# irwenqiang/DiFacto

Measured on AMD Instinct MI355X. Metric: train examples/sec (FM V_dim=16) at 1/8 GPU + achieved HBM GB/s, higher is better.
Workload: dtype f32; 1 GPU; C3 Criteo-shaped FM V_dim=16, 39 binary nnz/row, 2^24 keys, l1=0 V_threshold=0, fused dfx_train_step; config=c3, rows_per_gpu_step=100000, global_batch=100000, parallelism=single GPU

## Files before the change

### difacto_amd/_lib.py

```python
import ctypes
import os

import torch

LIB_PATH = os.environ.get("DFX_LIB_PATH") or os.path.join(
    os.path.dirname(os.path.abspath(__file__)), "libdifacto_amd.so")

_lib = None

c_i64 = ctypes.c_int64
c_u64 = ctypes.c_uint64
vp = ctypes.c_void_p
i64p = ctypes.POINTER(ctypes.c_int64)
f64p = ctypes.POINTER(ctypes.c_double)


class DfxError(RuntimeError):
    pass


class Batch(ctypes.Structure):
    _fields_ = [("size", c_i64), ("nnz", c_i64), ("offset", vp), ("index", vp), ("value", vp),
                ("label", vp), ("weight", vp)]


class Progress(ctypes.Structure):
    _fields_ = [("nrows", ctypes.c_double), ("loss", ctypes.c_double), ("auc", ctypes.c_double),
                ("penalty", ctypes.c_double), ("nnz_w", ctypes.c_double)]


class HostBatch(ctypes.Structure):
    _fields_ = [("offset", vp), ("index", vp), ("value", vp), ("label", vp), ("weight", vp),
                ("max_rows", c_i64), ("max_nnz", c_i64)]


_SIGS = {
    "dfx_last_error": (ctypes.c_char_p, []),
    "dfx_ctx_create": (ctypes.c_int, [ctypes.c_int, ctypes.c_char_p, ctypes.POINTER(vp)]),
    "dfx_ctx_destroy": (ctypes.c_int, [vp]),
    "dfx_ctx_set_stream": (ctypes.c_int, [vp, vp]),
    "dfx_ctx_use_own_stream": (ctypes.c_int, [vp]),
    "dfx_ctx_set_input_stream": (ctypes.c_int, [vp, vp]),
    "dfx_prof_lanes": (ctypes.c_int, [vp, f64p]),
    "dfx_prof_counts": (ctypes.c_int, [vp, f64p]),
    "dfx_prof_host": (ctypes.c_int, [vp, f64p]),
    "dfx_ctx_vdim": (ctypes.c_int, [vp]),
    "dfx_sync": (ctypes.c_int, [vp]),
    "dfx_malloc": (ctypes.c_int, [vp, ctypes.POINTER(vp), ctypes.c_size_t]),
    "dfx_free": (ctypes.c_int, [vp, vp]),
    "dfx_memcpy": (ctypes.c_int, [vp, vp, vp, ctypes.c_size_t, ctypes.c_int]),
    "dfx_reserve": (ctypes.c_int, [vp, c_i64, c_i64]),
    "dfx_localize": (ctypes.c_int, [vp, c_i64, c_i64, vp, vp, c_u64, vp, vp, vp, i64p]),
    "dfx_fm_predict": (ctypes.c_int, [vp, c_i64, c_i64, vp, vp, vp, vp, vp, vp, c_i64,
                                      ctypes.c_int, vp]),
    "dfx_fm_calcgrad": (ctypes.c_int, [vp, c_i64, c_i64, vp, vp, vp, vp, vp, vp, vp, vp, c_i64,
                                       ctypes.c_int, vp, vp]),
    "dfx_get_pos": (ctypes.c_int, [vp, c_i64, vp, vp, vp]),
    "dfx_evaluate": (ctypes.c_int, [vp, c_i64, vp, vp, f64p]),
    "dfx_auc": (ctypes.c_int, [vp, c_i64, vp, vp, f64p]),
    "dfx_store_pull": (ctypes.c_int, [vp, vp, c_i64, vp, vp, i64p]),
    "dfx_store_push": (ctypes.c_int, [vp, vp, c_i64, ctypes.c_int, vp, c_i64, vp]),
    "dfx_store_save": (ctypes.c_int, [vp, ctypes.c_char_p, ctypes.c_int]),
    "dfx_store_load": (ctypes.c_int, [vp, ctypes.c_char_p]),
    "dfx_store_load_part": (ctypes.c_int, [vp, ctypes.c_char_p, ctypes.c_int, ctypes.c_int]),
    "dfx_store_dump": (ctypes.c_int, [vp, ctypes.c_char_p, ctypes.c_int, ctypes.c_int]),
    "dfx_store_stats": (ctypes.c_int, [vp, i64p, i64p, f64p, ctypes.POINTER(ctypes.c_uint32)]),
    "dfx_store_evaluate": (ctypes.c_int, [vp, f64p, i64p]),
    "dfx_store_reserve": (ctypes.c_int, [vp, c_i64, c_i64]),
    "dfx_store_entry": (ctypes.c_int, [vp, c_u64, vp, vp, ctypes.POINTER(ctypes.c_int),
                                       ctypes.POINTER(ctypes.c_int)]),
    "dfx_train_step": (ctypes.c_int, [vp, ctypes.POINTER(Batch), ctypes.c_int, ctypes.c_int,
                                      c_u64, vp]),
    "dfx_progress_read": (ctypes.c_int, [vp, ctypes.POINTER(Progress), ctypes.c_int]),
    "dfx_prof_enable": (ctypes.c_int, [vp, ctypes.c_int]),
    "dfx_prof_enable_marks": (ctypes.c_int, [vp, ctypes.c_int, ctypes.c_uint]),
    "dfx_prof_read": (ctypes.c_int, [vp, f64p, ctypes.POINTER(ctypes.c_int), f64p]),
    "dfx_feeder_create": (ctypes.c_int, [vp, c_i64, c_i64, ctypes.POINTER(vp)]),
    "dfx_feeder_destroy": (ctypes.c_int, [vp]),
    "dfx_feeder_slot": (ctypes.c_int, [vp, ctypes.POINTER(HostBatch)]),
    "dfx_feeder_submit": (ctypes.c_int, [vp, c_i64, c_i64, ctypes.c_int, ctypes.c_int,
                                         ctypes.POINTER(Batch)]),
    "dfx_feeder_consumed": (ctypes.c_int, [vp]),
    "dfx_feeder_create_slots": (ctypes.c_int, [vp, c_i64, c_i64, ctypes.c_int,
                                               ctypes.POINTER(vp)]),
    "dfx_feeder_consumed_back": (ctypes.c_int, [vp, ctypes.c_int]),
    "dfx_dist_record_floats": (ctypes.c_int, [vp]),
    "dfx_dist_localize": (ctypes.c_int, [vp, ctypes.POINTER(Batch), c_u64, ctypes.c_int,
                                         ctypes.c_int, vp, vp]),
    "dfx_dist_localize_wait": (ctypes.c_int, [vp, ctypes.c_int, ctypes.c_int, i64p, i64p]),
    "dfx_dist_owner_begin": (ctypes.c_int, [vp, ctypes.c_int, vp, i64p, ctypes.c_int, vp]),
    "dfx_dist_owner_pull": (ctypes.c_int, [vp, ctypes.c_int, vp]),
    "dfx_dist_fwd_bwd": (ctypes.c_int, [vp, ctypes.c_int, ctypes.POINTER(Batch), vp,
                                        ctypes.c_int, vp, vp]),
    "dfx_dist_owner_push": (ctypes.c_int, [vp, ctypes.c_int, vp]),
    "dfx_dist_initv_local": (ctypes.c_int, [vp, ctypes.c_int, vp]),
    "dfx_dist_initv_draw": (ctypes.c_int, [vp, ctypes.c_int, vp, ctypes.c_int, ctypes.c_int]),
    "dfx_dist_push_agg_sum": (ctypes.c_int, [vp]),
    "dfx_store_probe_stats": (ctypes.c_int, [vp, vp, vp, vp]),
    "dfx_dist_union": (ctypes.c_int, [vp, vp, vp, ctypes.c_int, ctypes.c_int, vp, vp, vp, vp]),
    "dfx_dist_union_rows": (ctypes.c_int, [vp, vp, vp, ctypes.c_int64, vp, ctypes.c_int,
                                           ctypes.c_int64, ctypes.c_int, ctypes.c_int, vp, vp]),
    "dfx_split_part_floats": (ctypes.c_int, [vp, ctypes.c_int]),
    "dfx_split_pxv_floats": (ctypes.c_int, [vp]),
    "dfx_split_partition": (ctypes.c_int, [vp, ctypes.c_int, ctypes.POINTER(Batch), c_u64,
                                           ctypes.c_int, vp, vp, vp]),
    "dfx_split_partition_wait": (ctypes.c_int, [vp, ctypes.c_int, ctypes.c_int, i64p]),
    "dfx_split_owner_begin": (ctypes.c_int, [vp, ctypes.c_int, vp, vp, vp, i64p, i64p,
                                             ctypes.c_int, ctypes.c_int, ctypes.c_int,
                                             ctypes.c_int]),
    "dfx_ctx_lane_stream": (ctypes.c_int, [vp, ctypes.c_int, ctypes.POINTER(vp)]),
    "dfx_ctx_set_lane_stream": (ctypes.c_int, [vp, ctypes.c_int, vp]),
    "dfx_split_owner_forward": (ctypes.c_int, [vp, ctypes.c_int, vp]),
    "dfx_split_owner_forward_rows": (ctypes.c_int, [vp, ctypes.c_int, vp, ctypes.c_int, c_i64,
                                                    c_i64, c_i64]),
    "dfx_split_combine_rows": (ctypes.c_int, [vp, ctypes.c_int, ctypes.POINTER(Batch), vp, c_i64,
                                              ctypes.c_int, vp, vp, c_i64, c_i64]),
    "dfx_split_combine": (ctypes.c_int, [vp, ctypes.c_int, ctypes.POINTER(Batch), vp, c_i64,
                                         ctypes.c_int, vp, vp]),
    "dfx_split_owner_backward": (ctypes.c_int, [vp, ctypes.c_int, vp]),
    "dfx_split_owner_stats": (ctypes.c_int, [vp, ctypes.c_int, i64p, i64p, i64p]),
    "dfx_split_initv_local": (ctypes.c_int, [vp, ctypes.c_int, vp]),
    "dfx_split_initv_draw": (ctypes.c_int, [vp, ctypes.c_int, vp, ctypes.c_int, ctypes.c_int]),
}

EXPORTED = tuple(_SIGS)


def lib():
    global _lib
    if _lib is None:
        if not os.path.exists(LIB_PATH):
            raise DfxError("libdifacto_amd.so is not built (%s); run `make` at the repo root"
                           % LIB_PATH)
        L = ctypes.CDLL(LIB_PATH)
        lenient = bool(os.environ.get("DFX_LIB_PATH"))
        for name, (res, args) in _SIGS.items():
            if lenient and not hasattr(L, name):
                continue
            fn = getattr(L, name)
            fn.restype = res
            fn.argtypes = args
        _lib = L
    return _lib


def check(rc):
    if rc != 0:
        msg = lib().dfx_last_error()
        raise DfxError("libdifacto_amd: status %d: %s" % (rc, msg.decode() if msg else "?"))


DIST_PATH = os.path.join(os.path.dirname(os.path.abspath(LIB_PATH)), "libdfx_dist.so")
_dist = None
u32 = ctypes.c_uint32

_DIST_SIGS = {
    "dfx_dist_last_error": (ctypes.c_char_p, []),
    "dfx_dist_rccl_id_bytes": (ctypes.c_int, []),
    "dfx_dist_rccl_ids": (ctypes.c_int, [ctypes.c_int, vp]),
    "dfx_dist_rccl_comms": (ctypes.c_int, []),
    "dfx_split_store_set_slices": (ctypes.c_int, [vp, ctypes.c_int]),
    "dfx_split_store_allreduce_sum": (ctypes.c_int, [vp, f64p, ctypes.c_int]),
    "dfx_split_store_create_rccl": (ctypes.c_int, [vp, ctypes.c_int, ctypes.c_int, vp,
                                                   ctypes.c_int, ctypes.c_int, c_u64,
                                                   ctypes.POINTER(vp)]),
    "dfx_split_store_create_loopback": (ctypes.c_int, [ctypes.POINTER(vp), ctypes.c_int,
                                                       ctypes.c_int, c_u64, ctypes.POINTER(vp)]),
    "dfx_split_store_submit": (ctypes.c_int, [vp, ctypes.POINTER(Batch), ctypes.c_int,
                                              ctypes.c_int, ctypes.POINTER(vp)]),
    "dfx_split_store_flush": (ctypes.c_int, [vp]),
    "dfx_split_store_sync": (ctypes.c_int, [vp]),
    "dfx_split_store_throttle_seconds": (ctypes.c_int, [vp, f64p]),
    "dfx_split_store_set_marks": (ctypes.c_int, [vp, u32]),
    "dfx_split_store_take_marks": (ctypes.c_int, [vp, f64p, i64p]),
    "dfx_split_store_destroy": (ctypes.c_int, [vp]),
}

DIST_EXPORTED = tuple(_DIST_SIGS)


def dist_lib():
    global _dist
    if _dist is None:
        lib()
        if not os.path.exists(DIST_PATH):
            raise DfxError("libdfx_dist.so is not built (%s); run `make` at the repo root"
                           % DIST_PATH)
        L = ctypes.CDLL(DIST_PATH)
        for name, (res, args) in _DIST_SIGS.items():
            fn = getattr(L, name)
            fn.restype = res
            fn.argtypes = args
        _dist = L
    return _dist


def dist_check(rc):
    if rc != 0:
        msg = dist_lib().dfx_dist_last_error()
        raise DfxError("libdfx_dist: status %d: %s" % (rc, msg.decode() if msg else "?"))
```

### difacto_amd/csrc/internal.h

```cpp
#pragma once
#include <hip/hip_runtime.h>

#include <string>
#include <vector>

#include "../../include/difacto_amd.h"
#include "common.h"

namespace dfx {

void set_error(const std::string& msg);

#define DFX_HIP(call)                                                                 \
  do {                                                                                \
    hipError_t _e = (call);                                                           \
    if (_e != hipSuccess) {                                                           \
      ::dfx::set_error(std::string(#call) + ": " + hipGetErrorString(_e));            \
      return DFX_ERR_HIP;                                                             \
    }                                                                                 \
  } while (0)

#define DFX_CHECK_ARG(cond, msg)              \
  do {                                        \
    if (!(cond)) {                            \
      ::dfx::set_error(msg);                  \
      return DFX_ERR_ARG;                     \
    }                                         \
  } while (0)

#define DFX_TRY(expr)             \
  do {                            \
    int _rc = (expr);             \
    if (_rc != DFX_OK) return _rc; \
  } while (0)

struct DevBuf {
  void* p = nullptr;
  size_t bytes = 0;
  int ensure(size_t n);
  void release();
  template <typename T> T* as() const { return static_cast<T*>(p); }
};

constexpr int kBwStripes = 32;

struct DevState {
  unsigned long long n_keys;
  unsigned long long n_vrows;
  unsigned int seed;
  int err;
  long long new_w;
  double prog[5];
  unsigned long long or_mask;
  unsigned long long and_mask;
  unsigned long long diff_mask;
  unsigned int u_count;
  unsigned int n_init;
  unsigned int sortmeta[32];
  unsigned int totals[8];
  unsigned int sort_epoch;
  int probe_flag;
  double auc_n;
  double sum_u;
  double n_steps;
  unsigned long long live_keys;
  unsigned long long live_occ;
  double scratch[8];
  unsigned int iv_ticket;
  unsigned int iv_epoch;
  unsigned long long ivr_ticket[2];
  unsigned long long iv_done;
  long long iv_count;
  unsigned long long kmin, kmax, pk_min, pk_max;
  unsigned int pk_valid;
  unsigned int lb_over;
  unsigned int lb_sp_wbits, lb_sp_use, lb_hot;
  unsigned int lb_nhot, lb_hm_n, lb_hm_s;
  unsigned int lb_map_steps;
  unsigned long long lb_hm_base;
  alignas(128) unsigned long long bw_stripe[kBwStripes][16];
};

constexpr int kMaxDistRanks = 64;
constexpr int kSlots = 4;
inline bool any_pending(const bool (&v)[kSlots]) {
  for (bool b : v)
    if (b) return true;
  return false;
}
constexpr int kOsSortTile = 4096;
constexpr int kOsDigits = 8;
constexpr int kOsParts = 16;

struct Workspace {
  DevBuf keys0, keys1, vals0, vals1, rowid;
  DevBuf hist;
  DevBuf tiles;
  DevBuf uniq, cnt, segstart, col, slot, flags, wb, Vb, vpos;
  DevBuf occ_row, occ_x;
  DevBuf wv;
  DevBuf p, pred, XVp, rowtmp;
  DevBuf ak0, ak1, av0, av1;
  DevBuf dscratch;
  DevBuf ivstat;
  DevBuf live;
  DevBuf vlist;
  DevBuf hstat;
  DevBuf lbcnt, lbq, lbsplit, cptiles;
  unsigned int* lb_hint = nullptr;
  DevBuf os;
  int64_t os_tiles = 0;
  int os_reserve(int64_t ntiles, hipStream_t st);
  uint32_t* os_parts() const { return os.as<uint32_t>(); }
  uint32_t* os_counts() const { return os.as<uint32_t>() + kOsParts * kOsDigits * 256; }
  unsigned long long* os_status() const {
    return reinterpret_cast<unsigned long long*>(os.as<char>() + kOsCountBytes);
  }
  static constexpr size_t kOsCountBytes = (kOsParts + 1) * kOsDigits * 256 * sizeof(uint32_t);
  DevBuf oflags, ofrank, osegstart, osegslot, oseg_of, osorted;
  int64_t rows = 0, nnz = 0;
};

struct Context;

constexpr int kCapRing = 8;
struct CapGuard {
  hipEvent_t ev[kCapRing] = {};
  unsigned long long* host = nullptr;
  int64_t enq_at[kCapRing] = {};
  int head = 0, count = 0;
  int64_t enq_total = 0;
  int64_t known_keys = 0, known_vrows = 0, known_enq = 0;
};

struct Lane {
  hipStream_t stream;
  Workspace* ws;
  DevState* ds;
  int* err;
};

struct Context {
  int device = 0;
  hipStream_t stream = nullptr;
  hipStream_t own_stream = nullptr;
  Params P{};
  int loss_fm = 1;
  Table T{};
  int64_t cap = 0;
  DevState* ds = nullptr;
  float* zpad = nullptr;
  Workspace ws;
  std::vector<hipEvent_t> prof_ev;
  std::vector<hipEvent_t> lane_ev;
  double lane_stats[4] = {0, 0, 0, 0};
  int prof_max = 0, prof_n = 0;
  unsigned prof_mask = ~0u;
  Workspace ows[kSlots];
  DevState* ods[kSlots] = {};
  Workspace uws;
  int64_t dist_R[kSlots] = {}, dist_rows[kSlots] = {}, dist_U[kSlots] = {-1, -1, -1, -1};
  std::vector<int64_t> dist_offs[kSlots];
  bool dist_segs_pending[kSlots] = {};
  const uint64_t* dist_K[kSlots] = {};
  const uint32_t* dist_P[kSlots] = {};
  unsigned long long* dist_host[kSlots] = {};
  hipStream_t loc_stream = nullptr, aux_stream = nullptr;
  hipStream_t own_loc_stream = nullptr;
  hipStream_t part_stream = nullptr;
  hipStream_t own_part_stream = nullptr;
  hipStream_t in_stream = nullptr;
  bool has_in_stream = false;
  Workspace bws[kSlots];
  DevState* bds[kSlots] = {};
  Workspace aws;
  Workspace aws_alt;
  int auc_par = 0;
  hipEvent_t ev_auc_p[2] = {};
  DevState* ads = nullptr;
  hipEvent_t ev_in = nullptr, ev_fwd = nullptr, ev_auc = nullptr;
  hipEvent_t ev_loc[kSlots] = {}, ev_free[kSlots] = {};
  hipEvent_t slot_free[kSlots] = {};
  uint64_t auc_seq_p[2] = {};
  int split_auc_par = 0, split_auc_cur = 0;
  int split_auc_joined_par[kSlots] = {};
  uint64_t split_auc_joined[kSlots] = {};
  int parity = 0;
  long bwd_lds = -1;
  int autogrow = 1;
  int slot_es = 0;
  int fat_fwd = 1;
  int fwd_cpl = 8;
  int nt_mask = 0;
  int bwd_two_pass = 1;
  int bwd_cpl = 8;
  int bwd_cpl_from = 64;
  int loc_x_payload = 1;
  int lr_lanes = 1;
  int loc_bucket = 1;
  int lb_gather = 2;
  int lb_hnt = 0;
  int lb_diag = 0;
  int lb_skip = 0;
  int diag = 0;
  bool loc_done[2] = {false, false};
  const uint2* loc_rowof[2] = {nullptr, nullptr};
  int sort_pack = 1;
  int auc_sort = 1;
  CapGuard capg;
  double host_wait_s = 0;
  int64_t host_waits = 0;

  bool dist_live[kSlots] = {};
  bool dist_pushed[kSlots] = {};
  int dist_sum = 1;
  bool dist_initv_pending[kSlots] = {};
  int64_t split_B[kSlots] = {}, split_nblk[kSlots] = {};
  int64_t split_rows[kSlots] = {}, split_nnz[kSlots] = {};
  const uint64_t* split_keys[kSlots] = {};
  const float* split_x[kSlots] = {};
  bool split_resolved[kSlots] = {};
  bool split_initv_pending[kSlots] = {};
  bool split_initv_gated[kSlots] = {};
  bool split_lane[kSlots] = {};
  int split_job[kSlots] = {};
  hipEvent_t ev_part[kSlots] = {};
};

inline Lane main_lane(Context* c) { return Lane{c->stream, &c->ws, c->ds, &c->ds->err}; }

constexpr int kZpadFloats = 256 * 16 + 1024;

constexpr int kProfMarks = 8;
inline void lane_mark(Context* c, int m, hipStream_t st) {
  if (c->prof_n < c->prof_max && (c->prof_mask >> kProfMarks & 1u))
    (void)hipEventRecord(c->lane_ev[(size_t)c->prof_n * 4 + m], st);
}
inline void prof_mark(Context* c, int m) {
  if (c->prof_n < c->prof_max && (c->prof_mask >> m & 1u))
    (void)hipEventRecord(c->prof_ev[(size_t)c->prof_n * kProfMarks + m], c->stream);
}
inline hipEvent_t prof_mark_or(Context* c, int m, hipEvent_t other) {
  hipEvent_t e = other;
  if (c->prof_n < c->prof_max && (c->prof_mask >> m & 1u))
    e = c->prof_ev[(size_t)c->prof_n * kProfMarks + m];
  (void)hipEventRecord(e, c->stream);
  return e;
}

constexpr int kSortDiffIsOrAnd = 1, kSortCountsReady = 2;
inline constexpr int kSortPackRows(int rb8) { return rb8 << 8; }
inline constexpr int kSortItems(int it) { return it << 16; }
inline constexpr int kSortLookback(int lb) { return lb << 24; }
constexpr int kSortMetaPack = 25;
constexpr int kSortMetaEpoch = 24, kSortMetaHwTile = 26;
constexpr int kSortNT = 8;
__device__ inline bool sort_packed(const unsigned* meta) { return meta[kSortMetaPack] != 0u; }
__device__ inline void sort_unpack(const unsigned* meta, uint64_t and_mask, uint64_t w,
                                   uint64_t* key, uint32_t* row) {
  const unsigned pk = meta[kSortMetaPack];
  const int lo8 = (int)((pk >> 8) & 0xFFu), rb8 = (int)((pk >> 16) & 0xFFu);
  const uint64_t win = (rb8 == 0 ? ~0ull : (~0ull >> rb8)) << lo8;
  *key = (and_mask & ~win) | (((w >> rb8) << lo8) & win);
  *row = (uint32_t)(w & ((1ull << rb8) - 1));
}
__device__ inline uint64_t sort_key_bits(const unsigned* meta, uint64_t w) {
  const unsigned pk = meta[kSortMetaPack];
  return pk ? (w >> ((pk >> 16) & 0xFFu)) : w;
}
template <typename K, typename P>
int radix_sort_pairs(const Lane& L, K* k0, P* v0, K* k1, P* v1, int64_t n, int begin_bit,
                     int end_bit, const unsigned long long* diff_mask, unsigned int* sortmeta,
                     const uint32_t* n_dev = nullptr, int flags = 0);

void merge_runs(const Lane& L, std::vector<int64_t> runs, const uint64_t** K,
                const uint32_t** P);
constexpr int kMaxMergeRuns = 240;

int scan_u32(Context* c, uint32_t* data, int64_t n, uint32_t* total_dev,
             const uint32_t* n_dev = nullptr, const uint32_t* gate = nullptr);
int scan_u32(const Lane& L, uint32_t* data, int64_t n, uint32_t* total_dev,
             const uint32_t* n_dev = nullptr, const uint32_t* gate = nullptr);

constexpr int kChunkOcc = 128;
constexpr uint32_t kHotChunks = 8;
__host__ __device__ inline uint32_t hot_chunks_read(uint32_t nc) {
  return nc >= kHotChunks ? 1u : nc;
}
inline int64_t max_chunks(int64_t nnz) { return nnz / kChunkOcc + nnz / (kChunkOcc + 1) + 2; }
int chunk_plan(const Lane& L, int64_t nnz, const uint32_t* segstart, uint32_t* choff,
               uint32_t* chunk_seg, uint32_t* nchunks_dev);

void scan_tiles_top(const Lane& L, uint32_t* tilesum, int64_t ntiles, uint32_t* total_dev);
void scan_tiles_top_gated(const Lane& L, uint32_t* tilesum, int64_t ntiles, uint32_t* total_dev,
                          const uint32_t* gate);

constexpr int64_t kAucBlockMax = 12288;
struct LocOut {
  uint64_t* uniq = nullptr;
  float* cnt = nullptr;
  uint32_t* col = nullptr;
  bool col_heads = false;
  uint32_t* segstart = nullptr;
  const float* value = nullptr;
  uint32_t* occ_row = nullptr;
  float* occ_x = nullptr;
  bool keys_ready = false;
  const uint2** rowof_out = nullptr;
};
int localize_run(Context* c, const Lane& L, int64_t B, int64_t nnz, const uint64_t* offset,
                 const uint64_t* index, uint64_t max_index, const LocOut& o);
int localize_bucket(Context* c, const Lane& L, int64_t B, int64_t nnz, const uint64_t* offset,
                    const uint64_t* index, uint64_t max_index, const LocOut& o, bool* used);

int ws_reserve(Context* c, int64_t rows, int64_t nnz);
int pipeline_init(Context* c);
int table_unclump(Context* c);
int table_set_ranges(Context* c, int nranks);
int step_reserve(Context* c, int64_t rows, int64_t nnz);
int loc_reserve(Workspace& w, int64_t nnz, hipStream_t st);
int auc_reserve(Workspace& w, int64_t rows, hipStream_t st);

struct FinArgs {
  DevState* ds = nullptr;
  const DevState* bds = nullptr;
  int64_t B = 0;
  bool initv = false;
  int d = 0;
  int64_t vcap = 0;
  const double* loss_part = nullptr;
  int64_t nparts = 0;
  unsigned long long* cap_host = nullptr;
};
int run_initv(Context* c, int64_t n_bound, const uint32_t* flags, const uint32_t* slot,
              const DevState* nds = nullptr, const FinArgs* fin = nullptr);

__device__ inline void initv_advance(DevState* ds, int d, uint64_t draws, uint64_t rows,
                                     int64_t vcap) {
  ds->seed = lcg_advance(ds->seed, 3ull * (uint64_t)d * draws);
  const unsigned long long nv = ds->n_vrows + rows;
  ds->n_vrows = nv > (unsigned long long)vcap ? (unsigned long long)vcap : nv;
}

constexpr int kFinNT = 256;
template <int NT>
__device__ inline void step_finalize_body(const FinArgs& f, uint32_t initv_n, double* red) {
  DevState* ds = f.ds;
  unsigned long long snw = 0, snk = 0;
  if (threadIdx.x < kBwStripes) {
    unsigned long long* st = ds->bw_stripe[threadIdx.x];
    snw = st[0];
    snk = st[1];
    st[0] = 0ull;
    st[1] = 0ull;
  }
  if (threadIdx.x < kWave) {
    for (int off = 32; off > 0; off >>= 1) {
      snw += __shfl_xor(snw, off, kWave);
      snk += __shfl_xor(snk, off, kWave);
    }
  }
  double a = 0;
  for (int64_t i = threadIdx.x; i < f.nparts; i += NT) a += f.loss_part[i];
  for (int off = 32; off > 0; off >>= 1) a += __shfl_xor(a, off, kWave);
  if (lane_id() == 0) red[threadIdx.x / kWave] = a;
  __syncthreads();
  if (threadIdx.x != 0) return;
  double loss = 0;
  for (int k = 0; k < NT / kWave; ++k) loss += red[k];
  ds->scratch[3] = loss;
  ds->prog[0] += (double)f.B;
  ds->prog[1] += loss;
  ds->sum_u += (double)f.bds->u_count;
  ds->n_steps += 1;
  ds->n_init = 0;
  ds->iv_ticket = 0u;
  ds->iv_epoch += 1u;
  if (f.initv) initv_advance(ds, f.d, initv_n, initv_n, f.vcap);
  if (snw) atomicAdd((unsigned long long*)&ds->new_w, snw);
  if (snk) atomicAdd(&ds->n_keys, snk);
  if (f.cap_host) {
    f.cap_host[0] = ds->n_keys;
    f.cap_host[1] = ds->n_vrows;
  }
}

int push_cnt_seg_run(Context* c, int64_t n_bound, const uint32_t* segstart,
                     const uint32_t* segslot, uint32_t* flags, const DevState* nds);
int store_reserve(Context* c, int64_t n_keys, int64_t n_vrows);
int cap_check(Context* c, int64_t add);
int cap_record(Context* c);
int cap_record_slot(Context* c, unsigned long long** slot);
int cap_record_commit(Context* c, hipEvent_t* recorded = nullptr);
void cap_release(Context* c);
int store_maybe_grow(Context* c);

int initv_rank_count(const Lane& L, const uint32_t* flags, int64_t bound, const uint32_t* nuniq,
                     uint32_t* ftotal, const uint32_t* gate, int64_t* count_dev);
int initv_rank_draw(Context* c, const Lane& L, const uint32_t* flags, const uint32_t* ftotal,
                    const uint32_t* nuniq, int64_t bound, const uint32_t* segslot,
                    const int64_t* counts_all, int rank, int nranks, uint32_t* fcount,
                    unsigned long long* cap_host = nullptr);
int initv_by_rank(Context* c, const Lane& OL, int64_t R, int nranks, const uint32_t* segslot);
int push_cnt_seg_flags(Context* c, const Lane& L, int64_t n_bound, const uint32_t* segstart,
                       const uint32_t* segslot, uint32_t* flags, const DevState* nds);
int probe_keys_run(Context* c, const Lane& L, int64_t bound, const uint64_t* uniq,
                   uint32_t* segslot);
int auc_run(const Lane& L, int64_t B, const float* label, const float* pred, double* out_dev,
            int mode);
int auc_snapshot(const Lane& L, hipStream_t st, int64_t B, const float* label,
                 const float* pred);
int auc_finish(const Lane& L, int64_t B, double* out_dev, bool accumulate, int mode);
int evaluate_run(Context* c, int64_t B, const float* label, const float* pred, double* out_dev);

}

struct dfx_ctx {
  dfx::Context c;
};
```

### difacto_amd/csrc/locbucket.hip

```cpp
#include <algorithm>
#include <mutex>
#include <set>

#include "lookback.h"

namespace dfx {

constexpr int kLbNT = 256;
constexpr int kLbWaves = kLbNT / kWave;
constexpr int kLbCap = 2048;
constexpr int kLbMaxBits = 13;
constexpr int64_t kLbMaxRows = 2048;
constexpr int kLbIT = 8;
constexpr unsigned kLbOverRadix = 2;
constexpr unsigned kLbRetry = 64;
constexpr int kLbBigBlocks = 64;

struct LbArgs {
  int64_t B, nnz;
  const uint64_t* offset;
  const uint64_t* index;
  uint64_t max_index;
  int keys_ready;
  const float* value;
  int64_t rt, ntiles;
  int wbits;
  int nt;
  uint32_t* tilecnt;
  uint32_t* totals;
  uint32_t* bstart;
  uint32_t* bheads;
  uint32_t* brank;
  uint64_t* kbuf;
  uint32_t* qbuf;
  uint64_t* sbuf;
  uint2* rowof;
  uint64_t* kscr;
  uint32_t* qscr;
  uint64_t* sscr;
  DevState* ds;
  uint64_t* uniq;
  uint32_t* segstart;
  uint32_t* occ_row;
  float* occ_x;
  unsigned int* hint;
  int diag;
  uint64_t* hl_key;
  uint32_t* hl_len;
  uint64_t* hm_key;
  uint32_t* hm_p;
  uint32_t* hm_w;
  uint32_t* hm_ic;
  uint64_t* bfk;
  uint64_t* blk;
  uint32_t* bcont;
  int hm_lds;
  int wbits_hot;
  uint32_t hot_th;
};

__device__ inline uint64_t lb_key(uint64_t id, uint64_t max_index, int keys_ready) {
  if (keys_ready) return id;
  const uint64_t m = max_index == ~0ull ? (id == ~0ull ? 0ull : id) : id % max_index;
  return reverse_bytes(m);
}

__device__ inline int lb_bitlen(uint64_t x) { return x ? 64 - __clzll((long long)x) : 0; }

struct LbMap {
  uint64_t base;
  int s;
  uint32_t nbk;
};
__device__ inline LbMap lb_map(const DevState* ds, int wbits) {
  LbMap m;
  m.nbk = 1u << wbits;
  if (ds->pk_valid) {
    m.base = ds->pk_min;
    const int bl = lb_bitlen(ds->pk_max - ds->pk_min);
    m.s = bl > wbits ? bl - wbits : 0;
  } else {
    m.base = 0;
    m.s = 64 - wbits;
  }
  return m;
}
__device__ inline uint32_t lb_bucket(uint64_t k, const LbMap& m) {
  if (k <= m.base) return 0u;
  const uint64_t x = (k - m.base) >> m.s;
  return x < m.nbk ? (uint32_t)x : m.nbk - 1u;
}

constexpr int kLbHotMax = 1024;
struct LbHot {
  const uint64_t* hk;
  const uint32_t* hp;
  const uint32_t* hw;
  const uint32_t* ic;
  LbMap cm;
  double inv_nnz;
};
__device__ inline bool lb_hot_on(const LbArgs& a) {
  return a.hm_lds && a.value == nullptr && a.ds->lb_sp_use &&
         a.ds->lb_sp_wbits == (unsigned)a.wbits;
}
__host__ __device__ constexpr size_t lb_hot_lds(uint32_t nbk) {
  return (size_t)kLbHotMax * 8 + ((size_t)kLbHotMax + 1) * 4 + (size_t)kLbHotMax * 4 +
         ((size_t)nbk / 2 + 1) * 4;
}
__device__ inline LbHot lb_stage_hot(const LbArgs& a, void* lds, int t, int nt) {
  LbHot h;
  uint64_t* hk = reinterpret_cast<uint64_t*>(lds);
  uint32_t* hp = reinterpret_cast<uint32_t*>(hk + kLbHotMax);
  uint32_t* hw = hp + kLbHotMax + 1;
  uint32_t* ic = hw + kLbHotMax;
  const uint32_t n = a.ds->lb_hm_n, C = (1u << a.wbits) / 2;
  for (uint32_t i = t; i < n; i += nt) {
    hk[i] = a.hm_key[i];
    hw[i] = a.hm_w[i];
  }
  for (uint32_t i = t; i <= n; i += nt) hp[i] = a.hm_p[i];
  for (uint32_t c = t; c <= C; c += nt) ic[c] = a.hm_ic[c];
  h.hk = hk;
  h.hp = hp;
  h.hw = hw;
  h.ic = ic;
  h.cm.nbk = C;
  h.cm.base = a.ds->lb_hm_base;
  h.cm.s = (int)a.ds->lb_hm_s;
  h.inv_nnz = 1.0 / (double)a.nnz;
  return h;
}
__device__ inline uint32_t lb_hot_bucket(uint64_t k, uint64_t j, const LbHot& h) {
  const uint32_t c = lb_bucket(k, h.cm);
  uint32_t i = h.ic[c];
  const uint32_t i1 = h.ic[c + 1];
  for (; i < i1; ++i) {
    const uint64_t hkey = h.hk[i];
    if (hkey >= k) {
      if (hkey == k) {
        const uint32_t W = h.hw[i];
        uint32_t sub = (uint32_t)((double)j * (double)W * h.inv_nnz);
        sub = sub < W - 1 ? sub : W - 1;
        return c + h.hp[i] + 1 + sub;
      }
      break;
    }
  }
  return c + h.hp[i];
}

struct LbPack {
  uint64_t kmin;
  int lo, rb;
  bool packed;
};
__device__ inline LbPack lb_pack(const DevState* ds, uint64_t qmax) {
  LbPack p;
  p.kmin = ds->kmin;
  const uint64_t diff = ds->or_mask ^ ds->and_mask;
  p.lo = diff ? __ffsll((long long)diff) - 1 : 0;
  p.rb = lb_bitlen(qmax);
  p.packed = lb_bitlen((ds->kmax - ds->kmin) >> p.lo) + p.rb <= 63;
  return p;
}
__device__ inline uint64_t lb_keybits(const LbPack& p, uint64_t it) {
  return p.packed ? it >> p.rb : it;
}

__global__ void k_lb_init(DevState* ds) {
  ds->or_mask = 0;
  ds->and_mask = ~0ull;
  ds->kmin = ~0ull;
  ds->kmax = 0;
  ds->n_init = 0;
  ds->lb_over = 0;
  ds->lb_hot = 0;
  ds->lb_nhot = 0;
  unsigned* meta = ds->sortmeta;
  meta[kSortMetaEpoch] = ++ds->sort_epoch;
}

__device__ inline unsigned long long lb_wave_or(unsigned long long v) {
  for (int off = 32; off > 0; off >>= 1) v |= __shfl_xor(v, off, kWave);
  return v;
}
__device__ inline unsigned long long lb_wave_and(unsigned long long v) {
  for (int off = 32; off > 0; off >>= 1) v &= __shfl_xor(v, off, kWave);
  return v;
}
__device__ inline unsigned long long lb_wave_min(unsigned long long v) {
  for (int off = 32; off > 0; off >>= 1) {
    const unsigned long long o = __shfl_xor(v, off, kWave);
    v = o < v ? o : v;
  }
  return v;
}
__device__ inline unsigned long long lb_wave_max(unsigned long long v) {
  for (int off = 32; off > 0; off >>= 1) {
    const unsigned long long o = __shfl_xor(v, off, kWave);
    v = o > v ? o : v;
  }
  return v;
}

constexpr int kLbUnr = 8;


template <int HNT, bool HOT>
__global__ __launch_bounds__(HNT) void k_lb_hist(LbArgs a) {
  constexpr int kLbHNT = HNT, kLbHWaves = HNT / kWave;
  extern __shared__ uint64_t lb_dyn64[];
  uint32_t* hist = reinterpret_cast<uint32_t*>(lb_dyn64);
  __shared__ unsigned long long red[4][kLbHWaves];
  const LbMap m = lb_map(a.ds, a.wbits);
  const int t = threadIdx.x;
  for (uint32_t d = t; d < m.nbk; d += kLbHNT) hist[d] = 0;
  const bool qs = HOT && lb_hot_on(a);
  LbHot hm{};
  if (qs) hm = lb_stage_hot(a, hist + m.nbk, t, kLbHNT);
  const int64_t tile = blockIdx.x;
  const int64_t r0 = tile * a.rt;
  const int64_t r1 = r0 + a.rt < a.B ? r0 + a.rt : a.B;
  const uint64_t j0 = a.offset[r0], j1 = a.offset[r1];
  __syncthreads();
  unsigned long long vor = 0, vand = ~0ull, vmin = ~0ull, vmax = 0;
  for (uint64_t jb = j0; jb < j1; jb += (uint64_t)kLbUnr * kLbHNT) {
    uint64_t id[kLbUnr];
#pragma unroll
    for (int u = 0; u < kLbUnr; ++u) {
      const uint64_t j = jb + (uint64_t)u * kLbHNT + t;
      id[u] = j < j1 ? ldnt(a.index + j, a.nt != 0) : 0ull;
    }
#pragma unroll
    for (int u = 0; u < kLbUnr; ++u) {
      const uint64_t j = jb + (uint64_t)u * kLbHNT + t;
      if (j < j1) {
        const uint64_t k = lb_key(id[u], a.max_index, a.keys_ready);
        vor |= k;
        vand &= k;
        vmin = k < vmin ? k : vmin;
        vmax = k > vmax ? k : vmax;
        atomicAdd(&hist[qs ? lb_hot_bucket(k, j, hm) : lb_bucket(k, m)], 1u);
      }
    }
  }
  vor = lb_wave_or(vor);
  vand = lb_wave_and(vand);
  vmin = lb_wave_min(vmin);
  vmax = lb_wave_max(vmax);
  const int w = t / kWave;
  if (lane_id() == 0) {
    red[0][w] = vor;
    red[1][w] = vand;
    red[2][w] = vmin;
    red[3][w] = vmax;
  }
  __syncthreads();
  uint32_t* dst = a.tilecnt + (size_t)tile * m.nbk;
  for (uint32_t d = t; d < m.nbk; d += kLbHNT) dst[d] = hist[d];
  if (t == 0 && j1 > j0) {
    for (int i = 1; i < kLbHWaves; ++i) {
      vor |= red[0][i];
      vand &= red[1][i];
      vmin = red[2][i] < vmin ? red[2][i] : vmin;
      vmax = red[3][i] > vmax ? red[3][i] : vmax;
    }
    atomicOr(&a.ds->or_mask, vor);
    atomicAnd(&a.ds->and_mask, vand);
    atomicMin(&a.ds->kmin, vmin);
    atomicMax(&a.ds->kmax, vmax);
  }
}

constexpr int kLbScanWaves = 16;
__global__ __launch_bounds__(kLbScanWaves * kWave) void k_lb_colscan(LbArgs a) {
  __shared__ uint32_t part[kLbScanWaves][kWave];
  const int l = lane_id(), w = threadIdx.x / kWave;
  const uint32_t nbk = 1u << a.wbits;
  const uint32_t b = blockIdx.x * kWave + l;
  const bool ok = b < nbk;
  const int64_t T = a.ntiles, tt = (T + kLbScanWaves - 1) / kLbScanWaves;
  const int64_t t0 = (int64_t)w * tt < T ? (int64_t)w * tt : T;
  const int64_t t1 = t0 + tt < T ? t0 + tt : T;
  uint32_t s = 0;
  if (ok)
    for (int64_t i = t0; i < t1; ++i) s += a.tilecnt[(size_t)i * nbk + b];
  part[w][l] = s;
  __syncthreads();
  if (w == 0) {
    uint32_t run = 0;
    for (int i = 0; i < kLbScanWaves; ++i) {
      const uint32_t x = part[i][l];
      part[i][l] = run;
      run += x;
    }
    if (ok) {
      a.totals[b] = run;
      if (a.ds && run > (uint32_t)kLbCap) atomicAdd(&a.ds->lb_over, 1u);
    }
  }
  __syncthreads();
  if (ok) {
    uint32_t run = part[w][l];
    for (int64_t i = t0; i < t1; ++i) {
      uint32_t* p = a.tilecnt + (size_t)i * nbk + b;
      const uint32_t c = *p;
      *p = run;
      run += c;
    }
  }
}

template <bool S, int HNT, bool HOT>
__global__ __launch_bounds__(HNT) void k_lb_scatter(LbArgs a) {
  constexpr int kLbHNT = HNT, kLbHWaves = HNT / kWave;
  extern __shared__ uint64_t lb_dyn64[];
  __shared__ uint32_t lds[kLbHWaves + 1];
  __shared__ uint32_t whist[kLbHWaves][kWave];
  const LbMap m = lb_map(a.ds, a.wbits);
  uint32_t* cur = reinterpret_cast<uint32_t*>(lb_dyn64);
  uint64_t* offs = lb_dyn64 + (m.nbk + 1u) / 2;
  const int t = threadIdx.x;
  const bool qs = HOT && lb_hot_on(a);
  LbHot hm{};
  if (qs) hm = lb_stage_hot(a, offs + a.rt + 1, t, kLbHNT);
  const int64_t tile = ((a.diag & 512) && a.ntiles % 8 == 0)
                           ? (int64_t)(blockIdx.x % 8) * (a.ntiles / 8) + blockIdx.x / 8
                           : (int64_t)blockIdx.x;
  const int64_t r0 = tile * a.rt;
  const int nr = (int)(a.B - r0 < a.rt ? a.B - r0 : a.rt);
  const uint32_t per = (m.nbk + kLbHNT - 1) / kLbHNT;
  uint32_t mine = 0, over = 0;
  for (uint32_t i = 0; i < per; ++i) {
    const uint32_t d = t * per + i;
    if (d < m.nbk) {
      const uint32_t c = a.totals[d];
      mine += c;
      over += c > (uint32_t)kLbCap ? 1u : 0u;
    }
  }
  uint32_t total;
  uint32_t ex = block_excl_scan<kLbHNT>(mine, lds, &total);
  const uint32_t* pre = a.tilecnt + (size_t)tile * m.nbk;
  const bool mid4 = (a.diag & 512) && per == 4;
  uint32_t msum = 0;
  const uint32_t mex = ex;
  for (uint32_t i = 0; i < per; ++i) {
    const uint32_t d = t * per + i;
    if (d < m.nbk) {
      if (!mid4) cur[d] = ex + pre[d];
      msum += pre[d];
      if (blockIdx.x == 0) a.bstart[d] = ex;
      ex += a.totals[d];
    }
  }
  if (mid4) {
    __syncthreads();
    cur[t] = mex + msum;
  }
  if (a.diag & 256) {
    auto tcnt = [&](uint32_t d) {
      const uint32_t nx = tile + 1 < a.ntiles ? a.tilecnt[(size_t)(tile + 1) * m.nbk + d]
                                              : a.totals[d];
      return nx - pre[d];
    };
    uint32_t lm = 0;
    for (uint32_t i = 0; i < per; ++i)
      if (t * per + i < m.nbk) lm += tcnt(t * per + i);
    uint32_t lex = block_excl_scan<kLbHNT>(lm, lds, nullptr);
    for (uint32_t i = 0; i < per; ++i) {
      const uint32_t d = t * per + i;
      if (d < m.nbk) {
        const uint32_t cd = tcnt(d);
        cur[d] = lex;
        lex += cd;
      }
    }
  }
  const uint64_t qmax = (S || a.rowof) ? (uint64_t)(a.nnz - 1) : (uint64_t)(a.B - 1);
  const LbPack p = lb_pack(a.ds, qmax);
  if (blockIdx.x == 0) {
    uint32_t nover;
    (void)block_excl_scan<kLbHNT>(over, lds, &nover);
    if (t == 0) {
      a.bstart[m.nbk] = total;
      a.hint[0] = nover;
      a.hint[2] = p.packed ? 1u : 2u;
    }
  }
  for (int i = t; i <= nr; i += kLbHNT) offs[i] = a.offset[r0 + i];
  __syncthreads();
  const uint64_t j0 = offs[0], j1 = offs[nr];
  const uint64_t qmask = p.rb ? (~0ull >> (64 - p.rb)) : 0ull;
  const int w = t / kWave, l = lane_id();
  uint32_t* wh = whist[w];
  auto search = [&](uint64_t j) {
    int lo = 0, hi = (a.diag & 8) ? 0 : nr;
    while (hi - lo > 1) {
      const int mid = (lo + hi) >> 1;
      if (offs[mid] <= j) lo = mid; else hi = mid;
    }
    return lo;
  };
  for (uint64_t jb = j0; jb < j1; jb += (uint64_t)kLbUnr * kLbHNT) {
    const uint64_t wj = jb + (uint64_t)w * kLbUnr * kWave;
    uint64_t id[kLbUnr];
    float x[kLbUnr];
#pragma unroll
    for (int u = 0; u < kLbUnr; ++u) {
      const uint64_t j = wj + (uint64_t)u * kWave + l;
      id[u] = j < j1 ? ldnt(a.index + j, a.nt != 0) : 0ull;
      if (S) x[u] = j < j1 ? ldnt(a.value + j, a.nt != 0) : 0.f;
    }
    if (wj >= j1) continue;
    int ra = search(wj);
#pragma unroll
    for (int u = 0; u < kLbUnr; ++u) {
      const uint64_t J = wj + (uint64_t)u * kWave;
      if (J >= j1) break;
      const int rl = ra + 1 + l;
      const uint64_t sl = rl <= nr ? offs[rl] : ~0ull;
      wh[l] = 0;
      __builtin_amdgcn_wave_barrier();
      if (sl - J < (uint64_t)kWave) atomicAdd(&wh[sl - J], 1u);
      __builtin_amdgcn_wave_barrier();
      const uint32_t before = wave_incl_scan(wh[l]);
      __builtin_amdgcn_wave_barrier();
      const bool full = __shfl(sl, kWave - 1, kWave) <= J + kWave;
      const uint64_t j = J + l;
      const int lo = full ? search(j) : ra + (int)before;
      ra = full ? search(J + kWave)
                : ra + (int)__popcll(__ballot(sl <= J + kWave));
      if (j >= j1) continue;
      const uint64_t k = lb_key(id[u], a.max_index, a.keys_ready);
      const uint32_t row = (uint32_t)(r0 + lo);
      const uint64_t q = S ? j : (uint64_t)row;
      const uint32_t bk = qs ? lb_hot_bucket(k, j, hm) : lb_bucket(k, m);
      const uint32_t pos = atomicAdd(&cur[mid4 ? bk >> 2 : bk], 1u);
      stnt((a.diag & 128) ? a.sscr + j : (a.diag & (256 | 512)) ? a.sscr + (a.diag & 256 ? j0 : 0) + pos : a.kbuf + pos,
           p.packed ? ((((k - p.kmin) >> p.lo) << p.rb) | (q & qmask)) : k, a.nt != 0);
      if (!p.packed) a.qbuf[pos] = (uint32_t)q;
      if (S && a.rowof) a.rowof[j] = make_uint2(row, __float_as_uint(x[u]));
      else if (S) a.sbuf[pos] = (uint64_t)__float_as_uint(x[u]) | ((uint64_t)row << 32);
    }
  }
}

template <bool S>
__device__ void lb_global_pass(const uint64_t* Xk, const uint32_t* Xq, const uint64_t* Xs,
                               uint64_t* Yk, uint32_t* Yq, uint64_t* Ys, int64_t n, bool on_q,
                               int shift, uint32_t (*wcnt)[256], uint32_t* base, uint32_t* lds) {
  const int t = threadIdx.x, w = t / kWave, l = lane_id();
  base[t] = 0;
  __syncthreads();
  for (int64_t i = t; i < n; i += kLbNT) {
    const uint32_t d = on_q ? (Xq[i] >> shift) & 255u : (uint32_t)(Xk[i] >> shift) & 255u;
    atomicAdd(&base[d], 1u);
  }
  __syncthreads();
  {
    const uint32_t c = base[t];
    const uint32_t ex = block_excl_scan<kLbNT>(c, lds, nullptr);
    base[t] = ex;
  }
  __syncthreads();
  for (int64_t c0 = 0; c0 < n; c0 += (int64_t)kLbNT * kLbIT) {
    for (int i = t; i < kLbWaves * 256; i += kLbNT) (&wcnt[0][0])[i] = 0;
    __syncthreads();
    uint32_t dr[kLbIT];
    const int64_t wb = c0 + (int64_t)w * kWave * kLbIT;
#pragma unroll
    for (int j = 0; j < kLbIT; ++j) {
      const int64_t idx = wb + j * kWave + l;
      const bool valid = idx < n;
      const uint32_t d = !valid ? 0u
                         : on_q ? (Xq[idx] >> shift) & 255u
                                : (uint32_t)(Xk[idx] >> shift) & 255u;
      uint64_t peers = __ballot(valid);
#pragma unroll
      for (int bt = 0; bt < 8; ++bt) {
        const bool bit = (d >> bt) & 1u;
        const uint64_t mb = __ballot(valid && bit);
        peers &= bit ? mb : ~mb;
      }
      if (!valid) peers = 0;
      const uint32_t rk = (uint32_t)__popcll(peers & lanemask_lt());
      const uint32_t old = valid ? wcnt[w][d] : 0u;
      __builtin_amdgcn_wave_barrier();
      if (valid && rk == 0) wcnt[w][d] = old + (uint32_t)__popcll(peers);
      __builtin_amdgcn_wave_barrier();
      dr[j] = valid ? (d | ((old + rk) << 8)) : 0xFFFFFFFFu;
    }
    __syncthreads();
    {
      uint32_t run = base[t];
      for (int i = 0; i < kLbWaves; ++i) {
        const uint32_t x = wcnt[i][t];
        wcnt[i][t] = run;
        run += x;
      }
      base[t] = run;
    }
    __syncthreads();
#pragma unroll
    for (int j = 0; j < kLbIT; ++j) {
      if (dr[j] == 0xFFFFFFFFu) continue;
      const int64_t idx = wb + j * kWave + l;
      const uint32_t dst = wcnt[w][dr[j] & 255u] + (dr[j] >> 8);
      Yk[dst] = Xk[idx];
      if (Xq) Yq[dst] = Xq[idx];
      if (S) Ys[dst] = Xs[idx];
    }
    __syncthreads();
  }
  __threadfence();
  __syncthreads();
}

constexpr int kLbRadixIT = kLbCap / kLbNT;

template <bool Q, bool S>
__device__ inline void lb_lds_sort(uint64_t (&k)[kLbRadixIT], uint32_t (&q)[kLbRadixIT],
                                   uint64_t (&sv)[kLbRadixIT], int n, bool hasq,
                                   uint64_t* sk, uint32_t* sq, uint64_t* ss,
                                   uint32_t (*wcnt)[256], uint32_t* lds,
                                   unsigned long long (*red)[kLbWaves]) {
  const int t = threadIdx.x, w = t / kWave, l = lane_id();
  const int wb = w * kWave * kLbRadixIT;
  unsigned long long kor = 0, kand = ~0ull, qor = 0, qand = ~0ull;
#pragma unroll
  for (int c = 0; c < kLbRadixIT; ++c) {
    if (wb + c * kWave + l < n) {
      kor |= k[c];
      kand &= k[c];
      if (Q && hasq) {
        qor |= q[c];
        qand &= q[c];
      }
    }
  }
  kor = lb_wave_or(kor);
  kand = lb_wave_and(kand);
  if (Q) {
    qor = lb_wave_or(qor);
    qand = lb_wave_and(qand);
  }
  if (l == 0) {
    red[0][w] = kor;
    red[1][w] = kand;
    red[2][w] = qor;
    red[3][w] = qand;
  }
  __syncthreads();
  for (int i = 0; i < kLbWaves; ++i) {
    kor |= red[0][i];
    kand &= red[1][i];
    qor |= red[2][i];
    qand &= red[3][i];
  }
  const unsigned long long kvary = kor ^ kand, qvary = (Q && hasq) ? (qor ^ qand) : 0ull;
  int last = -1;
  for (int pass = 0; pass < 12; ++pass) {
    const unsigned long long vary = pass < 4 ? qvary : kvary;
    const int shift = 8 * (pass < 4 ? pass : pass - 4);
    if ((vary >> shift) & 255ull) last = pass;
  }
  if (last < 0) {
#pragma unroll
    for (int c = 0; c < kLbRadixIT; ++c) {
      const int idx = wb + c * kWave + l;
      if (idx < n) {
        sk[idx] = k[c];
        if (Q && hasq) sq[idx] = q[c];
        if (S) ss[idx] = sv[c];
      }
    }
    __syncthreads();
    return;
  }
  for (int pass = 0; pass <= last; ++pass) {
    const bool on_q = pass < 4;
    const unsigned long long vary = on_q ? qvary : kvary;
    const int shift = 8 * (on_q ? pass : pass - 4);
    if (((vary >> shift) & 255ull) == 0) continue;
#pragma unroll
    for (int i = 0; i < 256 / kWave; ++i) wcnt[w][i * kWave + l] = 0;
    __builtin_amdgcn_wave_barrier();
    uint32_t dr[kLbRadixIT];
#pragma unroll
    for (int c = 0; c < kLbRadixIT; ++c) {
      const bool valid = wb + c * kWave + l < n;
      const uint32_t d = !valid ? 0u : on_q ? (q[c] >> shift) & 255u
                                            : (uint32_t)(k[c] >> shift) & 255u;
      uint64_t peers = __ballot(valid);
#pragma unroll
      for (int bt = 0; bt < 8; ++bt) {
        const bool bit = (d >> bt) & 1u;
        const uint64_t mb = __ballot(valid && bit);
        peers &= bit ? mb : ~mb;
      }
      if (!valid) peers = 0;
      const uint32_t rk = (uint32_t)__popcll(peers & lanemask_lt());
      const uint32_t old = valid ? wcnt[w][d] : 0u;
      __builtin_amdgcn_wave_barrier();
      if (valid && rk == 0) wcnt[w][d] = old + (uint32_t)__popcll(peers);
      __builtin_amdgcn_wave_barrier();
      dr[c] = d | ((old + rk) << 8);
    }
    __syncthreads();
    {
      uint32_t run = 0;
#pragma unroll
      for (int i = 0; i < kLbWaves; ++i) {
        const uint32_t x = wcnt[i][t];
        wcnt[i][t] = run;
        run += x;
      }
      const uint32_t st = block_excl_scan<kLbNT>(run, lds, nullptr);
#pragma unroll
      for (int i = 0; i < kLbWaves; ++i) wcnt[i][t] += st;
    }
    __syncthreads();
#pragma unroll
    for (int c = 0; c < kLbRadixIT; ++c) {
      if (wb + c * kWave + l < n) {
        const uint32_t pos = wcnt[w][dr[c] & 255u] + (dr[c] >> 8);
        sk[pos] = k[c];
        if (Q && hasq) sq[pos] = q[c];
        if (S) ss[pos] = sv[c];
      }
    }
    __syncthreads();
    if (pass == last) break;
#pragma unroll
    for (int c = 0; c < kLbRadixIT; ++c) {
      const int idx = wb + c * kWave + l;
      if (idx < n) {
        k[c] = sk[idx];
        if (Q && hasq) q[c] = sq[idx];
        if (S) sv[c] = ss[idx];
      }
    }
    __syncthreads();
  }
}

__device__ inline bool lb_needs_global(int64_t n, bool packed, int q_lds) {
  return n > kLbCap || (!packed && !q_lds);
}

template <bool S>
__global__ __launch_bounds__(kLbNT) void k_lb_big(LbArgs a, int q_lds) {
  __shared__ uint32_t wcnt[kLbWaves][256];
  __shared__ uint32_t base[256];
  __shared__ uint32_t lds[kLbWaves + 1];
  __shared__ unsigned long long s_red[4][kLbWaves];
  const int t = threadIdx.x;
  const uint32_t nbk = 1u << a.wbits;
  const uint64_t qmax = (S || a.rowof) ? (uint64_t)(a.nnz - 1) : (uint64_t)(a.B - 1);
  const LbPack p = lb_pack(a.ds, qmax);
  const bool hasq = !p.packed;
  if (__hip_atomic_load(&a.ds->lb_over, __ATOMIC_RELAXED, __HIP_MEMORY_SCOPE_AGENT) == 0u &&
      (p.packed || q_lds))
    return;
  __shared__ uint32_t s_list[kLbNT];
  __shared__ uint32_t s_nlist;
  uint32_t listed = 0;
  for (uint32_t b0 = 0; b0 < nbk; b0 += kLbNT) {
    const uint32_t bb = b0 + t;
    const int64_t nb = bb < nbk ? (int64_t)a.bstart[bb + 1] - (int64_t)a.bstart[bb] : 0;
    const uint32_t need = (bb < nbk && nb > 1 && lb_needs_global(nb, p.packed, q_lds)) ? 1u : 0u;
    uint32_t cnt;
    const uint32_t ex = block_excl_scan<kLbNT>(need, lds, &cnt);
    if (t == 0) s_nlist = 0;
    __syncthreads();
    if (need && (listed + ex) % gridDim.x == blockIdx.x) s_list[atomicAdd(&s_nlist, 1u)] = bb;
    __syncthreads();
    listed += cnt;
    const uint32_t nl = s_nlist;
    for (uint32_t li = 0; li < nl; ++li) {
    const uint32_t b = s_list[li];
    const int64_t start = a.bstart[b];
    const int64_t n = (int64_t)a.bstart[b + 1] - start;
    unsigned long long kor = 0, kand = ~0ull, qor = 0, qand = ~0ull;
    for (int64_t i = t; i < n; i += kLbNT) {
      const uint64_t x = a.kbuf[start + i];
      kor |= x;
      kand &= x;
      if (hasq) {
        qor |= a.qbuf[start + i];
        qand &= a.qbuf[start + i];
      }
    }
    kor = lb_wave_or(kor);
    kand = lb_wave_and(kand);
    qor = lb_wave_or(qor);
    qand = lb_wave_and(qand);
    if (lane_id() == 0) {
      s_red[0][t / kWave] = kor;
      s_red[1][t / kWave] = kand;
      s_red[2][t / kWave] = qor;
      s_red[3][t / kWave] = qand;
    }
    __syncthreads();
    for (int i = 0; i < kLbWaves; ++i) {
      kor |= s_red[0][i];
      kand &= s_red[1][i];
      qor |= s_red[2][i];
      qand &= s_red[3][i];
    }
    __syncthreads();
    uint64_t* Xk = a.kbuf + start;
    uint32_t* Xq = hasq ? a.qbuf + start : nullptr;
    uint64_t* Xs = S ? a.sbuf + start : nullptr;
    uint64_t* Yk = a.kscr + start;
    uint32_t* Yq = hasq ? a.qscr + start : nullptr;
    uint64_t* Ys = S ? a.sscr + start : nullptr;
    int np = 0;
    for (int pass = 0; pass < 12; ++pass) {
      const bool on_q = pass < 4;
      const int shift = 8 * (on_q ? pass : pass - 4);
      const unsigned long long vary = on_q ? (hasq ? (qor ^ qand) : 0ull) : (kor ^ kand);
      if (((vary >> shift) & 255ull) == 0) continue;
      lb_global_pass<S>(Xk, Xq, Xs, Yk, Yq, Ys, n, on_q, shift, wcnt, base, lds);
      uint64_t* tk = Xk; Xk = Yk; Yk = tk;
      uint32_t* tq = Xq; Xq = Yq; Yq = tq;
      uint64_t* ts = Xs; Xs = Ys; Ys = ts;
      ++np;
    }
    if (np & 1) {
      for (int64_t i = t; i < n; i += kLbNT) {
        Yk[i] = Xk[i];
        if (hasq) Yq[i] = Xq[i];
        if (S) Ys[i] = Xs[i];
      }
    }
    __syncthreads();
    }
    __syncthreads();
  }
}

constexpr int kLbWIT = kLbCap / kWave;


template <bool Q, bool S>
__device__ __attribute__((always_inline)) inline void lb_wave_sort(
    const uint64_t* gk, const uint32_t* gq, const uint64_t* gs, int n, bool hasq, int ntp,
    int diag, uint64_t* sk, uint32_t* sq, uint64_t* ss, uint32_t* cnt) {
  const int l = threadIdx.x;
  const int nc = (n + kWave - 1) / kWave;
  uint64_t k[kLbWIT], sv[kLbWIT];
  uint32_t q[kLbWIT];
#pragma unroll
  for (int c = 0; c < kLbWIT; ++c) {
    const int i = c * kWave + l;
    const bool v = c < nc && i < n;
    k[c] = v ? ldnt(gk + i, ntp != 0) : ~0ull;
    q[c] = (Q && hasq) ? (v ? gq[i] : ~0u) : 0u;
    sv[c] = (S && v) ? gs[i] : 0ull;
  }
  unsigned long long kor = 0, kand = ~0ull, qor = 0, qand = ~0ull;
#pragma unroll
  for (int c = 0; c < kLbWIT; ++c) {
    if (c < nc) {
      kor |= k[c] == ~0ull ? 0ull : k[c];
      kand &= k[c];
      if (Q && hasq) {
        qor |= q[c] == ~0u ? 0u : q[c];
        qand &= q[c];
      }
    }
  }
  kor = lb_wave_or(kor);
  kand = lb_wave_and(kand);
  if (Q) {
    qor = lb_wave_or(qor);
    qand = lb_wave_and(qand);
  }
  const unsigned long long kvary = kor ^ kand, qvary = (Q && hasq) ? (qor ^ qand) : 0ull;
  auto passes = [&]() {
    auto pass_at = [&](int pass, bool* on_q, int* shift) {
      *on_q = pass < 4;
      *shift = 8 * (*on_q ? pass : pass - 4);
      return true;
    };
    int last = -1;
    if (!(diag & 1))
      for (int pass = 0; pass < 12; ++pass) {
        bool on_q;
        int shift;
        if (!pass_at(pass, &on_q, &shift)) break;
        if (((on_q ? qvary : kvary) >> shift) & 255ull) last = pass;
      }
    if (last < 0) {
#pragma unroll
      for (int c = 0; c < kLbWIT; ++c) {
        if (c < nc) {
          const int i = c * kWave + l;
          sk[i] = k[c];
          if (Q && hasq) sq[i] = q[c];
          if (S) ss[i] = sv[c];
        }
      }
    }
    for (int pass = 0; pass <= last; ++pass) {
      bool on_q;
      int shift;
      (void)pass_at(pass, &on_q, &shift);
      const unsigned long long vary = on_q ? qvary : kvary;
      if (((vary >> shift) & 255ull) == 0) continue;
#pragma unroll
      for (int i = 0; i < 256 / kWave; ++i) cnt[i * kWave + l] = 0;
      __builtin_amdgcn_wave_barrier();
#pragma unroll
      for (int c = 0; c < kLbWIT; ++c) {
        if (c < nc) {
          const uint32_t d = on_q ? (q[c] >> shift) & 255u : (uint32_t)(k[c] >> shift) & 255u;
          atomicAdd(&cnt[d], 1u);
        }
      }
      __builtin_amdgcn_wave_barrier();
      {
        const uint32_t c0 = cnt[4 * l], c1 = cnt[4 * l + 1], c2 = cnt[4 * l + 2],
                       c3 = cnt[4 * l + 3];
        const uint32_t s4 = c0 + c1 + c2 + c3;
        const uint32_t ex = wave_incl_scan(s4) - s4;
        __builtin_amdgcn_wave_barrier();
        cnt[4 * l] = ex;
        cnt[4 * l + 1] = ex + c0;
        cnt[4 * l + 2] = ex + c0 + c1;
        cnt[4 * l + 3] = ex + c0 + c1 + c2;
        __builtin_amdgcn_wave_barrier();
      }
      uint32_t pos[kLbWIT];
#pragma unroll
      for (int c = 0; c < kLbWIT; ++c) {
        pos[c] = 0;
        if (c < nc) {
          const uint32_t d = on_q ? (q[c] >> shift) & 255u : (uint32_t)(k[c] >> shift) & 255u;
          uint64_t peers = ~0ull;
#pragma unroll
          for (int bt = 0; bt < 8; ++bt) {
            const bool bit = (d >> bt) & 1u;
            const uint64_t mb = __ballot(bit);
            peers &= bit ? mb : ~mb;
          }
          const uint32_t rk = (uint32_t)__popcll(peers & lanemask_lt());
          const uint32_t base = cnt[d];
          __builtin_amdgcn_wave_barrier();
          if (rk == 0) cnt[d] = base + (uint32_t)__popcll(peers);
          __builtin_amdgcn_wave_barrier();
          pos[c] = base + rk;
        }
      }
#pragma unroll
      for (int c = 0; c < kLbWIT; ++c) {
        if (c < nc) {
          sk[pos[c]] = k[c];
          if (Q && hasq) sq[pos[c]] = q[c];
          if (S) ss[pos[c]] = sv[c];
        }
      }
      __builtin_amdgcn_wave_barrier();
      if (pass == last) break;
#pragma unroll
      for (int c = 0; c < kLbWIT; ++c) {
        if (c < nc) {
          const int i = c * kWave + l;
          k[c] = sk[i];
          if (Q && hasq) q[c] = sq[i];
          if (S) sv[c] = ss[i];
        }
      }
      __builtin_amdgcn_wave_barrier();
    }
    __builtin_amdgcn_wave_barrier();
  };
  passes();
}

template <bool Q, bool S>
__global__ __launch_bounds__(kWave) void k_lb_wbucket(LbArgs a) {
  __shared__ uint64_t sk[kLbCap];
  __shared__ uint32_t sq[Q ? kLbCap : 1];
  __shared__ uint64_t ss[S ? kLbCap : 1];
  __shared__ uint32_t cnt[256];
  DevState* ds = a.ds;
  const int l = threadIdx.x;
  const uint32_t b = blockIdx.x;
  const int64_t start = a.bstart[b];
  const int n = (int)((int64_t)a.bstart[b + 1] - start);
  const uint64_t qmax = (S || a.rowof) ? (uint64_t)(a.nnz - 1) : (uint64_t)(a.B - 1);
  const LbPack p = lb_pack(ds, qmax);
  const bool hasq = !p.packed;
  const bool fast = !lb_needs_global(n, p.packed, Q ? 1 : 0);
  const uint64_t* gk = a.kbuf + start;
  const uint32_t* gq = a.qbuf + start;
  const uint64_t* gs = a.sbuf + start;
  const int nc = (n + kWave - 1) / kWave;
  if (fast)
    lb_wave_sort<Q, S>(gk, gq, gs, n, hasq, a.nt, a.diag, sk, sq, ss, cnt);
  const uint64_t qmask = p.rb ? (~0ull >> (64 - p.rb)) : 0ull;
  uint32_t* tseg = a.qscr + start;
  uint64_t* tkey = a.kscr + start;
  uint32_t run = 0;
  bool longseg = false, hot = false;
  const int th = (int)a.hot_th;
  auto fullkey = [&](uint64_t it) { return p.packed ? (((it >> p.rb) << p.lo) + p.kmin) : it; };
  auto heads = [&](const uint64_t* K, const uint32_t* Qs, const uint64_t* Ss) {
    uint64_t prev = 0;
    for (int c = 0; c < nc; ++c) {
      const int i = c * kWave + l;
      const bool valid = i < n;
      const uint64_t it = valid ? K[i] : 0ull;
      const uint64_t kb = lb_keybits(p, it);
      const uint64_t up = __shfl_up(kb, 1, kWave);
      const bool h = valid && (i == 0 || kb != (l == 0 ? prev : up));
      if (valid && i >= kChunkOcc && kb == lb_keybits(p, K[i - kChunkOcc])) longseg = true;
      if (longseg && valid && i >= th && kb == lb_keybits(p, K[i - th])) hot = true;
      prev = __shfl(kb, kWave - 1, kWave);
      const uint64_t hb = __ballot(h);
      if (!(a.diag & 4) && valid) {
        if (h) {
          const uint32_t r = run + (uint32_t)__popcll(hb & lanemask_lt());
          tkey[r] = fullkey(it);
          tseg[r] = (uint32_t)(start + i);
        }
        uint32_t row;
        if (S) {
          const uint64_t sw = Ss[i];
          row = (uint32_t)(sw >> 32);
          if (a.occ_x) a.occ_x[start + i] = __uint_as_float((uint32_t)sw);
        } else if (a.rowof) {
          row = p.packed ? (uint32_t)(it & qmask) : Qs[i];
        } else {
          row = p.packed ? (uint32_t)(it & qmask) : Qs[i];
        }
        a.occ_row[start + i] = row;
      }
      run += (uint32_t)__popcll(hb);
    }
  };
  if (fast) heads(sk, sq, ss);
  else heads(gk, gq, gs);
  if (n > 0 && l == 0) {
    a.bfk[b] = fullkey(fast ? sk[0] : gk[0]);
    a.blk[b] = fullkey(fast ? sk[n - 1] : gk[n - 1]);
  }
  if (__ballot(hot) && l == 0 &&
      __hip_atomic_load(&ds->lb_hot, __ATOMIC_RELAXED, __HIP_MEMORY_SCOPE_AGENT) == 0u)
    atomicOr(&ds->lb_hot, 1u);
  if (__ballot(longseg) && l == 0 &&
      __hip_atomic_load(&ds->n_init, __ATOMIC_RELAXED, __HIP_MEMORY_SCOPE_AGENT) == 0u)
    atomicOr(&ds->n_init, 1u);
  if (l == 0) a.bheads[b] = run;
}

constexpr int kLbScanNT = 1024;
__global__ __launch_bounds__(kLbScanNT) void k_lb_bscan(LbArgs a) {
  __shared__ uint32_t lds[kLbScanNT / kWave + 1];
  __shared__ int s_last[kLbScanNT];
  const int t = threadIdx.x;
  const uint32_t nbk = 1u << a.wbits;
  const uint32_t per = (nbk + kLbScanNT - 1) / kLbScanNT;
  const bool hm = lb_hot_on(a);
  int lastne = -1;
  for (uint32_t i = 0; hm && i < per; ++i) {
    const uint32_t d = t * per + i;
    if (d < nbk && a.bstart[d + 1] > a.bstart[d]) lastne = (int)d;
  }
  s_last[t] = lastne;
  __syncthreads();
  for (int off = 1; hm && off < kLbScanNT; off <<= 1) {
    const int v = t >= off ? s_last[t - off] : -1;
    __syncthreads();
    if (v > s_last[t]) s_last[t] = v;
    __syncthreads();
  }
  int prev = t > 0 && hm ? s_last[t - 1] : -1;
  uint32_t mine = 0, anycont = 0;
  for (uint32_t i = 0; i < per; ++i) {
    const uint32_t d = t * per + i;
    if (d < nbk) {
      uint32_t c = 0;
      if (hm && a.bstart[d + 1] > a.bstart[d]) {
        if (prev >= 0 && a.bfk[d] == a.blk[prev]) c = 1;
        prev = (int)d;
      }
      a.bcont[d] = c;
      anycont |= c;
      mine += a.bheads[d] - c;
    }
  }
  uint32_t U;
  uint32_t ex = block_excl_scan<kLbScanNT>(mine, lds, &U);
  for (uint32_t i = 0; i < per; ++i) {
    const uint32_t d = t * per + i;
    if (d < nbk) {
      a.brank[d] = ex;
      ex += a.bheads[d] - a.bcont[d];
    }
  }
  if (anycont && __hip_atomic_load(&a.ds->n_init, __ATOMIC_RELAXED, __HIP_MEMORY_SCOPE_AGENT) == 0u)
    atomicOr(&a.ds->n_init, 1u);
  if (t == 0) {
    DevState* ds = a.ds;
    ds->u_count = U;
    if (a.segstart) a.segstart[U] = (uint32_t)a.nnz;
    ds->pk_min = ds->kmin;
    ds->pk_max = ds->kmax;
    ds->pk_valid = 1u;
  }
}

__global__ __launch_bounds__(kLbNT) void k_lb_out(LbArgs a) {
  const uint32_t b = blockIdx.x;
  const int64_t start = a.bstart[b];
  const uint32_t h = a.bheads[b], r0 = a.brank[b], c = a.bcont[b];
  for (uint32_t j = threadIdx.x + c; j < h; j += kLbNT) {
    if (a.uniq) a.uniq[r0 + j - c] = a.kscr[start + j];
    if (a.segstart) a.segstart[r0 + j - c] = a.qscr[start + j];
  }
}

constexpr int kLbHotGrid = 512;
__global__ __launch_bounds__(kLbNT) void k_lb_hotlist(LbArgs a) {
  DevState* ds = a.ds;
  if (ds->lb_hot == 0u && !lb_hot_on(a)) return;
  const int64_t U = ds->u_count;
  for (int64_t i = (int64_t)blockIdx.x * kLbNT + threadIdx.x; i < U;
       i += (int64_t)gridDim.x * kLbNT) {
    const uint32_t len = a.segstart[i + 1] - a.segstart[i];
    if (len >= a.hot_th) {
      const uint32_t x = atomicAdd(&ds->lb_nhot, 1u);
      if (x < (uint32_t)kLbHotMax) {
        a.hl_key[x] = a.uniq[i];
        a.hl_len[x] = len;
      }
    }
  }
}

__global__ __launch_bounds__(kLbHotMax) void k_lb_hotmap(LbArgs a) {
  __shared__ uint64_t sk[kLbHotMax];
  __shared__ uint32_t sl[kLbHotMax];
  __shared__ uint32_t lds[kLbHotMax / kWave + 1];
  DevState* ds = a.ds;
  const int t = threadIdx.x;
  const bool was = lb_hot_on(a);
  const uint32_t nh = (ds->lb_hot || was) ? ds->lb_nhot : 0u;
  if (t == 0 && was) ds->lb_map_steps += 1u;
  const int wb = a.wbits_hot;
  const uint32_t nbk = 1u << wb, C = nbk / 2;
  if (nh == 0u || nh > (uint32_t)kLbHotMax || wb < 2 || 2 * nh >= nbk - C) {
    if (t == 0) {
      ds->lb_sp_use = 0u;
      a.hint[3] = 0u;
    }
    return;
  }
  sk[t] = (uint32_t)t < nh ? a.hl_key[t] : ~0ull;
  sl[t] = (uint32_t)t < nh ? a.hl_len[t] : 0u;
  __syncthreads();
  {
    const uint64_t mk = sk[t];
    const uint32_t ml = sl[t];
    uint32_t r = 0;
    if ((uint32_t)t < nh)
      for (uint32_t i = 0; i < nh; ++i) r += sk[i] < mk ? 1u : 0u;
    __syncthreads();
    if ((uint32_t)t < nh) {
      sk[r] = mk;
      sl[r] = ml;
    }
    __syncthreads();
  }
  const uint32_t len = sl[t];
  uint32_t mass;
  (void)block_excl_scan<kLbHotMax>(len, lds, &mass);
  const uint32_t room = nbk - C - 2 * nh;
  const uint32_t target = (mass + room - 1) / room;
  const uint32_t W = (uint32_t)t < nh ? (len + target - 1) / target : 0u;
  uint32_t tot;
  const uint32_t P = block_excl_scan<kLbHotMax>((uint32_t)t < nh ? W + 1 : 0u, lds, &tot);
  if ((uint32_t)t < nh) {
    a.hm_key[t] = sk[t];
    a.hm_w[t] = W;
    a.hm_p[t] = P;
  }
  if (t == 0) a.hm_p[nh] = tot;
  LbMap cm;
  cm.nbk = C;
  cm.base = ds->kmin;
  {
    const int bl = lb_bitlen(ds->kmax - ds->kmin), cb = wb - 1;
    cm.s = bl > cb ? bl - cb : 0;
  }
  for (uint32_t c = t; c <= C; c += kLbHotMax) {
    uint32_t lo = 0, hi = nh;
    while (lo < hi) {
      const uint32_t mid = (lo + hi) >> 1;
      if (lb_bucket(sk[mid], cm) < c) lo = mid + 1;
      else hi = mid;
    }
    a.hm_ic[c] = lo;
  }
  if (t == 0) {
    ds->lb_hm_n = nh;
    ds->lb_hm_base = cm.base;
    ds->lb_hm_s = (unsigned)cm.s;
    ds->lb_sp_wbits = (unsigned)wb;
    ds->lb_sp_use = 1u;
    a.hint[3] = 1u;
    if (!was) a.hint[0] = 0u;
  }
}

__global__ __launch_bounds__(kLbNT) void k_lb_gather(LbArgs a) {
  const int64_t i = (int64_t)blockIdx.x * kLbNT + threadIdx.x;
  if (i >= a.nnz) return;
  const uint2 rv = a.rowof[a.occ_row[i]];
  a.occ_row[i] = rv.x;
  if (a.occ_x) a.occ_x[i] = __uint_as_float(rv.y);
}

static size_t lb_split_bytes() {
  constexpr size_t kNb = (size_t)1 << kLbMaxBits;
  return (size_t)kLbHotMax * 8 * 2 + kNb * 8 * 2 + (size_t)kLbHotMax * 4 * 3 + 4 + (kNb / 2 + 1) * 4 +
         kNb * 4;
}

static void lb_lds_attr(const void* f) {
  static std::mutex mu;
  static std::set<const void*> done;
  std::lock_guard<std::mutex> g(mu);
  if (!done.insert(f).second) return;
  hipFuncAttributes at{};
  if (hipFuncGetAttributes(&at, f) == hipSuccess)
    (void)hipFuncSetAttribute(f, hipFuncAttributeMaxDynamicSharedMemorySize,
                              160 * 1024 - (int)at.sharedSizeBytes);
  (void)hipGetLastError();
}

int localize_bucket(Context* c, const Lane& L, int64_t B, int64_t nnz, const uint64_t* offset,
                    const uint64_t* index, uint64_t max_index, const LocOut& o, bool* used) {
  *used = false;
  Workspace& ws = *L.ws;
  if (!ws.lb_hint) {
    DFX_HIP(hipHostMalloc(reinterpret_cast<void**>(&ws.lb_hint), 4 * sizeof(unsigned int),
                          hipHostMallocDefault));
    for (int i = 0; i < 4; ++i) ws.lb_hint[i] = 0;
  }
  volatile unsigned int* hint = ws.lb_hint;
  if (hint[0] > kLbOverRadix) {
    if (++hint[1] < kLbRetry) return DFX_OK;
    hint[0] = 0;
    hint[1] = 0;
  }
  const bool valued = o.value != nullptr && o.occ_x != nullptr;
  int wbits = 1;
  while (wbits < kLbMaxBits && ((int64_t)1024 << wbits) < nnz) ++wbits;
  uint32_t nbk = 1u << wbits;
  if (nnz > (int64_t)nbk * (kLbCap * 3 / 4)) return DFX_OK;
  if (hint[2] == 0u) {
    int kb = 64;
    if (!o.keys_ready && max_index != ~0ull) {
      kb = 0;
      for (uint64_t m = max_index - 1; m; m >>= 8) kb += 8;
    }
    const uint64_t qmax = valued ? (uint64_t)(nnz - 1) : (uint64_t)(B - 1);
    int rb = 0;
    for (uint64_t q = qmax; q; q >>= 1) ++rb;
    hint[2] = kb + rb <= 63 ? 1u : 2u;
  }
  const int hm_lds = (!valued && hint[3]) ? 1 : 0;
  const int wbits_key = wbits, wbits_hot = wbits + 1 < kLbMaxBits ? wbits + 1 : kLbMaxBits;
  if (hm_lds) {
    wbits = wbits_hot;
    nbk = 1u << wbits;
  }
  constexpr int64_t kLbTiles = 128;
  int64_t ntiles = std::min<int64_t>(kLbTiles, std::max<int64_t>(1, nnz / 4096));
  int64_t rt = std::min<int64_t>(kLbMaxRows, std::max<int64_t>(1, (B + ntiles - 1) / ntiles));
  ntiles = (B + rt - 1) / rt;
  DFX_TRY(ws.keys0.ensure(nnz * 8));
  DFX_TRY(ws.keys1.ensure(nnz * 8));
  DFX_TRY(ws.vals0.ensure(nnz * 8));
  DFX_TRY(ws.vals1.ensure(nnz * 8));
  DFX_TRY(ws.lbq.ensure(nnz * 8));
  DFX_TRY(ws.lbcnt.ensure(sizeof(uint32_t) * ((size_t)ntiles * nbk + 4 * (nbk + 1))));
  DFX_TRY(ws.lbsplit.ensure(lb_split_bytes()));
  LbArgs a{};
  a.B = B; a.nnz = nnz; a.offset = offset; a.index = index; a.max_index = max_index;
  a.keys_ready = o.keys_ready ? 1 : 0;
  a.value = valued ? o.value : nullptr;
  a.rt = rt; a.ntiles = ntiles; a.wbits = wbits;
  a.nt = (c->nt_mask & kNtLane) ? 1 : 0;
  a.tilecnt = ws.lbcnt.as<uint32_t>();
  a.totals = a.tilecnt + (size_t)ntiles * nbk;
  a.bstart = a.totals + nbk + 1;
  a.bheads = a.bstart + nbk + 1;
  a.brank = a.bheads + nbk + 1;
  a.kbuf = ws.keys0.as<uint64_t>();
  a.kscr = ws.keys1.as<uint64_t>();
  a.sbuf = ws.vals0.as<uint64_t>();
  const bool gather = valued && c->lb_gather;
  a.rowof = gather ? ws.vals0.as<uint2>() : nullptr;
  a.sscr = ws.vals1.as<uint64_t>();
  a.qbuf = ws.lbq.as<uint32_t>();
  a.qscr = a.qbuf + nnz;
  a.ds = L.ds;
  a.uniq = o.uniq; a.segstart = o.segstart; a.occ_row = o.occ_row;
  a.occ_x = valued ? o.occ_x : nullptr;
  a.hint = ws.lb_hint;
  a.diag = (c->lb_diag & ~(16 | 32 | 64 | 128 | 256 | 512)) | c->lb_skip;
  {
    constexpr size_t kNb = (size_t)1 << kLbMaxBits;
    char* q = ws.lbsplit.as<char>();
    a.hl_key = reinterpret_cast<uint64_t*>(q);
    a.hm_key = a.hl_key + kLbHotMax;
    a.bfk = a.hm_key + kLbHotMax;
    a.blk = a.bfk + kNb;
    a.hl_len = reinterpret_cast<uint32_t*>(a.blk + kNb);
    a.hm_p = a.hl_len + kLbHotMax;
    a.hm_w = a.hm_p + kLbHotMax + 1;
    a.hm_ic = a.hm_w + kLbHotMax;
    a.bcont = a.hm_ic + kNb / 2 + 1;
  }
  a.hm_lds = hm_lds;
  a.wbits_hot = wbits_hot;
  a.hot_th = (uint32_t)std::max<int64_t>(
      kWave, std::min<int64_t>(nnz / ((int64_t)1 << wbits_key) / 2, kLbCap));
  const size_t sp_bytes = a.hm_lds ? lb_hot_lds(nbk) : 0;
  hipLaunchKernelGGL(k_lb_init, dim3(1), dim3(1), 0, L.stream, L.ds);
#define DFX_LB_HIST(NT)                                                                     \
  if (a.hm_lds) {                                                                           \
    lb_lds_attr((const void*)k_lb_hist<NT, true>);                                          \
    hipLaunchKernelGGL((k_lb_hist<NT, true>), dim3((unsigned)ntiles), dim3(NT),             \
                       nbk * sizeof(uint32_t) + sp_bytes, L.stream, a);                     \
  } else {                                                                                  \
    hipLaunchKernelGGL((k_lb_hist<NT, false>), dim3((unsigned)ntiles), dim3(NT),            \
                       nbk * sizeof(uint32_t), L.stream, a);                                \
  }
  const int hnt = c->lb_hnt ? c->lb_hnt : (valued ? 512 : 1024);
  if (hnt == 256) { DFX_LB_HIST(256) }
  else if (hnt == 512) { DFX_LB_HIST(512) }
  else { DFX_LB_HIST(1024) }
#undef DFX_LB_HIST
  hipLaunchKernelGGL(k_lb_colscan, dim3((nbk + kWave - 1) / kWave), dim3(kLbScanWaves * kWave), 0,
                     L.stream, a);
  const size_t scatter_lds =
      ((nbk + 1) & ~1u) * sizeof(uint32_t) + (rt + 1) * sizeof(uint64_t) + sp_bytes;
#define DFX_LB_SCAT(NT)                                                                    \
  lb_lds_attr((const void*)k_lb_scatter<true, NT, false>);                                 \
  lb_lds_attr((const void*)k_lb_scatter<false, NT, false>);                                \
  lb_lds_attr((const void*)k_lb_scatter<false, NT, true>);                                 \
  if (valued)                                                                              \
    hipLaunchKernelGGL((k_lb_scatter<true, NT, false>), dim3((unsigned)ntiles), dim3(NT),   \
                       scatter_lds, L.stream, a);                                          \
  else if (a.hm_lds)                                                                       \
    hipLaunchKernelGGL((k_lb_scatter<false, NT, true>), dim3((unsigned)ntiles), dim3(NT),   \
                       scatter_lds, L.stream, a);                                          \
  else                                                                                     \
    hipLaunchKernelGGL((k_lb_scatter<false, NT, false>), dim3((unsigned)ntiles), dim3(NT),  \
                       scatter_lds, L.stream, a);
  if (c->lb_skip & 16) {}
  else if (hnt == 256) { DFX_LB_SCAT(256) }
  else if (hnt == 512) { DFX_LB_SCAT(512) }
  else { DFX_LB_SCAT(1024) }
#undef DFX_LB_SCAT
  const bool q_lds = hint[2] == 2u;
  const dim3 bg(nbk), bb(kLbNT);
  const bool carry = valued && !gather;
  if (carry)
    hipLaunchKernelGGL(k_lb_big<true>, dim3(kLbBigBlocks), bb, 0, L.stream, a, q_lds ? 1 : 0);
  else
    hipLaunchKernelGGL(k_lb_big<false>, dim3(kLbBigBlocks), bb, 0, L.stream, a, q_lds ? 1 : 0);
  const dim3 wb(kWave);
  if (c->lb_skip & 32) {}
  else if (carry) {
    if (q_lds) hipLaunchKernelGGL((k_lb_wbucket<true, true>), bg, wb, 0, L.stream, a);
    else hipLaunchKernelGGL((k_lb_wbucket<false, true>), bg, wb, 0, L.stream, a);
  } else {
    if (q_lds) hipLaunchKernelGGL((k_lb_wbucket<true, false>), bg, wb, 0, L.stream, a);
    else hipLaunchKernelGGL((k_lb_wbucket<false, false>), bg, wb, 0, L.stream, a);
  }
  const bool defer = gather && c->lb_gather == 2 && o.rowof_out != nullptr;
  if (o.rowof_out) *o.rowof_out = defer ? a.rowof : nullptr;
  if (gather && !defer && nnz > 0)
    hipLaunchKernelGGL(k_lb_gather, dim3((unsigned)((nnz + kLbNT - 1) / kLbNT)), bb, 0, L.stream,
                       a);
  hipLaunchKernelGGL(k_lb_bscan, dim3(1), dim3(kLbScanNT), 0, L.stream, a);
  if (!(c->lb_skip & 64)) hipLaunchKernelGGL(k_lb_out, bg, bb, 0, L.stream, a);
  if (!valued && a.uniq && a.segstart) {
    hipLaunchKernelGGL(k_lb_hotlist, dim3(kLbHotGrid), bb, 0, L.stream, a);
    hipLaunchKernelGGL(k_lb_hotmap, dim3(1), dim3(kLbHotMax), 0, L.stream, a);
  }
  DFX_HIP(hipGetLastError());
  *used = true;
  return DFX_OK;
}

}
```

### difacto_amd/csrc/step.hip

```cpp

#include "fm_args.h"

namespace dfx {
void sum_parts(Context* c, const double* part, int64_t n, double* out, bool accumulate);
}

namespace dfx {

int xvp_stride(const Context* c) {
  const int d = c->P.V_dim;
  return (d > 0 && d % 32 != 0) ? (d + 1 + 31) / 32 * 32 : d;
}

int ws_reserve(Context* c, int64_t rows, int64_t nnz) {
  Workspace& ws = c->ws;
  const int d = c->P.V_dim;
  if (rows < 1) rows = 1;
  if (nnz < 1) nnz = 1;
  DFX_TRY(ws.flags.ensure((nnz + 1) * 4));
  DFX_TRY(ws.tiles.ensure(sizeof(uint32_t) * ((nnz + 2047) / 2048 + 1)));
  DFX_TRY(ws.p.ensure(rows * 4));
  DFX_TRY(ws.pred.ensure(rows * 4));
  if (d > 0) DFX_TRY(ws.XVp.ensure((size_t)rows * xvp_stride(c) * 4));
  DFX_TRY(ws.dscratch.ensure((rows / 4 + 64) * 8));
  DFX_TRY(ws.wv.ensure(nnz * 8));
  DFX_TRY(ws.Vb.ensure((size_t)max_chunks(nnz) * (d + 2) * 8));
  ws.rows = rows;
  ws.nnz = nnz;
  return DFX_OK;
}

int loc_reserve(Workspace& w, int64_t nnz, hipStream_t st) {
  if (nnz < 1) nnz = 1;
  DFX_TRY(w.keys0.ensure(nnz * 8));
  DFX_TRY(w.keys1.ensure(nnz * 8));
  DFX_TRY(w.vals0.ensure(nnz * 8));
  DFX_TRY(w.vals1.ensure(nnz * 8));
  DFX_TRY(w.os_reserve((nnz + 2047) / 2048, st));
  DFX_TRY(w.tiles.ensure(sizeof(uint32_t) * ((nnz + 2047) / 2048 + 1)));
  DFX_TRY(w.segstart.ensure((nnz + 1) * 4));
  DFX_TRY(w.col.ensure(nnz * 4));
  DFX_TRY(w.uniq.ensure(nnz * 8));
  DFX_TRY(w.flags.ensure((nnz + 1) * 4));
  DFX_TRY(w.rowtmp.ensure(max_chunks(nnz) * 4));
  DFX_TRY(w.slot.ensure((nnz + 1) * 4));
  DFX_TRY(w.occ_row.ensure(nnz * 4));
  DFX_TRY(w.occ_x.ensure(nnz * 4));
  w.nnz = nnz;
  return DFX_OK;
}

int auc_reserve(Workspace& w, int64_t rows, hipStream_t st) {
  if (rows < 1) rows = 1;
  if (w.rows >= rows && w.ak0.p) return DFX_OK;
  DFX_TRY(w.ak0.ensure(rows * 4));
  DFX_TRY(w.av0.ensure(rows * 4));
  DFX_TRY(w.keys0.ensure(rows * 8));
  DFX_TRY(w.keys1.ensure(rows * 8));
  DFX_TRY(w.vals0.ensure(rows * 4));
  DFX_TRY(w.vals1.ensure(rows * 4));
  DFX_TRY(w.os_reserve((rows + 2047) / 2048, st));
  w.rows = rows;
  return DFX_OK;
}

static bool auc_db_on(const Context*, int64_t) { return true; }

int step_reserve(Context* c, int64_t rows, int64_t nnz) {
  DFX_TRY(pipeline_init(c));
  DFX_TRY(ws_reserve(c, rows, nnz));
  DFX_TRY(loc_reserve(c->bws[0], nnz, c->loc_stream));
  DFX_TRY(loc_reserve(c->bws[1], nnz, c->loc_stream));
  if (auc_db_on(c, rows)) DFX_TRY(auc_reserve(c->aws_alt, rows, c->aux_stream));
  return auc_reserve(c->aws, rows, c->aux_stream);
}

constexpr int kProbeNT = 256, kProbeUnr = 4;
__global__ __launch_bounds__(kProbeNT) void k_probe_keys(const uint64_t* __restrict__ uniq,
                                                         const DevState* nds, Table T,
                                                         int2* __restrict__ pulled,
                                                         uint32_t* __restrict__ segslot,
                                                         DevState* ds) {
  __shared__ int red[kProbeNT / kWave];
  const int64_t n = (int64_t)nds->u_count;
  const int64_t ub = (int64_t)blockIdx.x * kProbeNT * kProbeUnr + threadIdx.x;
  uint64_t key[kProbeUnr], h[kProbeUnr];
  unsigned long long kk[kProbeUnr];
  int2 wr[kProbeUnr];
  int ins = 0;
#pragma unroll
  for (int v = 0; v < kProbeUnr; ++v) {
    const int64_t u = ub + (int64_t)v * kProbeNT;
    key[v] = u < n ? uniq[u] : 0ull;
    h[v] = tbl_hash(key[v], T);
  }
#pragma unroll
  for (int v = 0; v < kProbeUnr; ++v) {
    const int64_t u = ub + (int64_t)v * kProbeNT;
    if (u < n) {
      kk[v] = ent_at(T, h[v])->key;
      wr[v] = *reinterpret_cast<const int2*>(ent_at(T, h[v]));
    }
  }
#pragma unroll
  for (int v = 0; v < kProbeUnr; ++v) {
    const int64_t u = ub + (int64_t)v * kProbeNT;
    if (u >= n) continue;
    int64_t s = (int64_t)h[v];
    if (kk[v] != key[v]) {
      bool inserted;
      s = tbl_insert(T, key[v], &inserted);
      ins += inserted ? 1 : 0;
      if (s < 0) {
        atomicOr(&ds->err, insert_error(s));
        wr[v] = make_int2(0, -1);
      } else {
        wr[v] = *reinterpret_cast<const int2*>(ent_at(T, s));
      }
    }
    segslot[u] = s < 0 ? kNoSlot : (uint32_t)s;
    if (pulled) pulled[u] = wr[v];
  }
  for (int off = 32; off > 0; off >>= 1) ins += __shfl_xor(ins, off, kWave);
  if (lane_id() == 0) red[threadIdx.x / kWave] = ins;
  __syncthreads();
  if (threadIdx.x == 0) {
    int t = 0;
    for (int i = 0; i < kProbeNT / kWave; ++i) t += red[i];
    if (t) atomicAdd(&ds->n_keys, (unsigned long long)t);
  }
}

int probe_keys_run(Context* c, const Lane& L, int64_t bound, const uint64_t* uniq,
                   uint32_t* segslot) {
  if (bound <= 0) return DFX_OK;
  const dim3 ug((unsigned)((bound + kProbeNT * kProbeUnr - 1) / (kProbeNT * kProbeUnr)));
  hipLaunchKernelGGL(k_probe_keys, ug, dim3(kProbeNT), 0, L.stream, uniq, L.ds, c->T, nullptr,
                     segslot, c->ds);
  DFX_HIP(hipGetLastError());
  return DFX_OK;
}


__global__ __launch_bounds__(kFinNT) void k_step_finalize(FinArgs f) {
  __shared__ double red[kFinNT / kWave];
  step_finalize_body<kFinNT>(f, 0u, red);
}

__global__ __launch_bounds__(kWave) void k_fold_stripes(DevState* ds) {
  unsigned long long nw = 0, nk = 0;
  if (threadIdx.x < kBwStripes) {
    unsigned long long* st = ds->bw_stripe[threadIdx.x];
    nw = st[0];
    nk = st[1];
    st[0] = 0ull;
    st[1] = 0ull;
  }
  for (int off = 32; off > 0; off >>= 1) {
    nw += __shfl_xor(nw, off, kWave);
    nk += __shfl_xor(nk, off, kWave);
  }
  if (threadIdx.x == 0) {
    if (nw) atomicAdd((unsigned long long*)&ds->new_w, nw);
    if (nk) atomicAdd(&ds->n_keys, nk);
  }
}

static int fold_stripes_on_error(Context* c, int rc) {
  hipLaunchKernelGGL(k_fold_stripes, dim3(1), dim3(kWave), 0, c->stream, c->ds);
  (void)hipGetLastError();
  return rc;
}

int train_step(Context* c, const dfx_batch* b, int job_type, int push_cnt, uint64_t max_index,
               float* pred_out) {
  const int64_t B = b->size, nnz = b->nnz;
  const int d = c->P.V_dim;
  DFX_TRY(step_reserve(c, B, nnz));
  DFX_TRY(cap_check(c, nnz));
  Workspace& ws = c->ws;
  const int k = c->parity;
  c->parity ^= 1;
  Workspace& bw = c->bws[k];
  DevState* bds = c->bds[k];
  const Lane LL{c->loc_stream, &bw, bds, &c->ds->err};
  const bool db = auc_db_on(c, B);
  const int ap = db ? c->auc_par : 0;
  Workspace& aw = ap ? c->aws_alt : c->aws;
  hipEvent_t ev_auc_mine = db ? c->ev_auc_p[ap] : c->ev_auc;
  if (db) c->auc_par ^= 1;
  const Lane AL{c->aux_stream, &aw, c->ads, &c->ds->err};
  uint32_t* segstart = bw.segstart.as<uint32_t>();
  uint64_t* uniq = bw.uniq.as<uint64_t>();
  uint32_t* segslot = bw.slot.as<uint32_t>();
  uint32_t* occ_row = bw.occ_row.as<uint32_t>();
  float* occ_x = b->value ? bw.occ_x.as<float>() : nullptr;
  uint32_t* flags = ws.flags.as<uint32_t>();
  float* pred = pred_out ? pred_out : ws.pred.as<float>();

  DFX_HIP(hipEventRecord(c->ev_in, c->has_in_stream ? c->in_stream : c->stream));
  DFX_HIP(hipStreamWaitEvent(c->loc_stream, c->ev_in, 0));
  DFX_HIP(hipStreamWaitEvent(c->loc_stream, c->slot_free[k] ? c->slot_free[k] : c->ev_free[k], 0));
  LocOut o;
  o.segstart = segstart;
  o.value = b->value;
  o.occ_row = occ_row;
  o.occ_x = occ_x;
  o.col = nullptr;
  o.uniq = uniq;
  const uint2* rowof = c->loc_rowof[k];
  o.rowof_out = &rowof;
  lane_mark(c, 0, c->loc_stream);
  uint32_t* choff = bw.flags.as<uint32_t>();
  uint32_t* chunk_seg = bw.rowtmp.as<uint32_t>();
  uint32_t* nchunks = &bds->totals[1];
  if (!((c->diag & 2) && c->loc_done[k])) {
    rowof = nullptr;
    c->lb_skip = c->loc_done[k] ? (c->lb_diag & (16 | 32 | 64 | 128 | 256 | 512)) : 0;
    DFX_TRY(localize_run(c, LL, B, nnz, b->offset, b->index, max_index, o));
    c->lb_skip = 0;
    c->loc_rowof[k] = rowof;
    DFX_TRY(chunk_plan(LL, nnz, segstart, choff, chunk_seg, nchunks));
    c->loc_done[k] = true;
  }
  lane_mark(c, 1, c->loc_stream);
  DFX_HIP(hipStreamWaitEvent(c->loc_stream, ev_auc_mine, 0));
  DFX_HIP(hipEventRecord(c->ev_loc[k], c->loc_stream));

  const bool cnt_first = push_cnt && d > 0;
  const bool bwd_inserts = !cnt_first && job_type == DFX_JOB_TRAINING &&
                           B > 0 && nnz > 0;
  prof_mark(c, 0);
  DFX_HIP(hipStreamWaitEvent(c->stream, c->ev_loc[k], 0));
  prof_mark(c, 1);
  const dim3 ug((unsigned)((nnz + kProbeNT * kProbeUnr - 1) / (kProbeNT * kProbeUnr)));
  if (nnz > 0 && !bwd_inserts)
    hipLaunchKernelGGL(k_probe_keys, ug, dim3(kProbeNT), 0, c->stream, uniq, bds, c->T,
                       nullptr, segslot, c->ds);
  prof_mark(c, 2);
  if (cnt_first) {
    DFX_TRY(push_cnt_seg_run(c, nnz, segstart, segslot, flags, bds));
  }
  prof_mark(c, 3);

  FwdArgs a{};
  a.B = B; a.offs = b->offset; a.val = b->value;
  a.index = b->index; a.max_index = max_index;
  a.T = c->T; a.l1_shrk = c->P.l1_shrk; a.Vbase = c->T.V; a.zpad = c->zpad;
  a.no_fat_fwd = !c->fat_fwd;
  a.cpl = c->fwd_cpl;
  a.lr_lanes = c->lr_lanes;
  a.nt = c->nt_mask;
  a.d = d; a.label = b->label; a.rw = b->weight; a.pred = pred; a.p_out = ws.p.as<float>();
  a.XVp = ws.XVp.as<float>(); a.xs = xvp_stride(c);
  a.loss_part = ws.dscratch.as<double>() + 8;
  a.auc_key = aw.ak0.as<uint32_t>();
  a.auc_lab = aw.av0.as<uint32_t>();
  int nblk = 0;
  DFX_TRY(launch_fwd_fused(a, c->stream, &nblk, true));
  prof_mark(c, 4);

  auto auc_lane = [&]() -> int {
    const hipEvent_t e = prof_mark_or(c, 5, c->ev_fwd);
    DFX_HIP(hipStreamWaitEvent(c->aux_stream, e, 0));
    lane_mark(c, 2, c->aux_stream);
    if (!(c->diag & 1)) DFX_TRY(auc_finish(AL, B, &c->ds->prog[2], true, c->auc_sort));
    lane_mark(c, 3, c->aux_stream);
    DFX_HIP(hipEventRecord(c->ev_auc, c->aux_stream));
    DFX_HIP(hipEventRecord(c->ev_auc_p[ap], c->aux_stream));
    ++c->auc_seq_p[ap];
    return DFX_OK;
  };

  const bool bwd_runs = job_type == DFX_JOB_TRAINING && B > 0 && nnz > 0;
  const bool initv = bwd_runs && d > 0;
  FinArgs fin;
  fin.ds = c->ds; fin.bds = bds; fin.B = B; fin.initv = initv;
  fin.d = d; fin.vcap = c->T.vcap; fin.loss_part = a.loss_part; fin.nparts = nblk;
  if (bwd_runs) {
    BwdArgs g{};
    g.segstart = segstart; g.ds = bds; g.nseg_host = -1; g.segcol = nullptr;
    g.occ_row = occ_row; g.occ_x = occ_x; g.occ_rx = rowof; g.zpad = c->zpad;
    g.p = ws.p.as<float>();
    g.XVp = ws.XVp.as<float>(); g.xs = xvp_stride(c); g.d = d; g.slot = segslot;
    g.T = c->T; g.Pm = c->P;  g.cpl = c->bwd_cpl; g.cpl_from = c->bwd_cpl_from; g.nt = c->nt_mask;
    g.flags = flags; g.dsw = c->ds; g.stripes = &c->ds->bw_stripe[0][0];
    g.uniq = uniq; g.insert_keys = bwd_inserts ? 1 : 0;
    g.choff = choff; g.chunk_seg = chunk_seg; g.nchunks = nchunks; g.part = ws.Vb.as<double>();
    const bool count_live = c->prof_n < c->prof_max && (c->prof_mask >> 9 & 1u);
    DFX_TRY(bwd_two_pass_reserve(c, ws, nnz, &g));
    const int64_t nbb = bwd_fused_blocks(d, nnz, g.vlist != nullptr, g.cpl | g.cpl_from << 8);
    if (count_live) {
      DFX_TRY(ws.live.ensure((size_t)nbb * sizeof(uint2)));
      g.live_part = ws.live.as<uint2>();
    }
    DFX_TRY(launch_bwd_chunks(g, max_chunks(nnz), c->stream, true));
    DFX_TRY(auc_lane());
    DFX_TRY(launch_bwd_fused(g, nnz, c->stream, c->bwd_lds));
    if (count_live) DFX_TRY(sum_live(g.live_part, nbb, c->ds, c->stream));
    prof_mark(c, 6);
  } else {
    DFX_TRY(auc_lane());
    prof_mark(c, 6);
  }
  {
    const int rc = cap_record_slot(c, &fin.cap_host);
    if (rc != DFX_OK) return bwd_runs ? fold_stripes_on_error(c, rc) : rc;
  }
  if (initv) {
    const int rc = run_initv(c, nnz, flags, segslot, bds, &fin);
    if (rc != DFX_OK) return fold_stripes_on_error(c, rc);
  } else {
    hipLaunchKernelGGL(k_step_finalize, dim3(1), dim3(kFinNT), 0, c->stream, fin);
  }
  hipEvent_t fe = nullptr;
  DFX_TRY(cap_record_commit(c, &fe));
  if (!fe) {
    DFX_HIP(hipEventRecord(c->ev_free[k], c->stream));
    fe = c->ev_free[k];
  }
  c->slot_free[k] = fe;
  prof_mark(c, 7);
  if (c->prof_n < c->prof_max) ++c->prof_n;
  DFX_HIP(hipGetLastError());
  return DFX_OK;
}

}

using namespace dfx;

extern "C" int dfx_train_step(dfx_ctx* ctx, const dfx_batch* batch, int job_type, int push_cnt,
                              uint64_t max_index, float* pred_out) {
  DFX_CHECK_ARG(ctx && batch, "null argument");
  DFX_CHECK_ARG(batch->size >= 0 && batch->nnz >= 0, "train_step: negative sizes");
  DFX_CHECK_ARG(batch->size == 0 || (batch->offset && batch->label), "train_step: null buffer");
  DFX_CHECK_ARG(batch->nnz == 0 || batch->index, "train_step: null index");
  DFX_CHECK_ARG(job_type == DFX_JOB_TRAINING || job_type == DFX_JOB_VALIDATION ||
                    job_type == DFX_JOB_PREDICTION,
                "train_step: bad job type");
  return train_step(&ctx->c, batch, job_type, push_cnt, max_index, pred_out);
}

extern "C" int dfx_prof_enable(dfx_ctx* ctx, int max_steps) {
  return dfx_prof_enable_marks(ctx, max_steps, ~0u);
}

extern "C" int dfx_prof_enable_marks(dfx_ctx* ctx, int max_steps, unsigned mask) {
  DFX_CHECK_ARG(ctx && max_steps >= 0, "bad argument");
  Context* c = &ctx->c;
  c->prof_mask = mask;
  DFX_HIP(hipStreamSynchronize(c->stream));
  for (hipEvent_t e : c->prof_ev) (void)hipEventDestroy(e);
  c->prof_ev.assign((size_t)max_steps * kProfMarks, nullptr);
  for (auto& e : c->prof_ev) DFX_HIP(hipEventCreate(&e));
  for (hipEvent_t e : c->lane_ev) (void)hipEventDestroy(e);
  c->lane_ev.assign((size_t)max_steps * 4, nullptr);
  for (auto& e : c->lane_ev) DFX_HIP(hipEventCreate(&e));
  c->prof_max = max_steps;
  c->prof_n = 0;
  return DFX_OK;
}

extern "C" int dfx_prof_counts(dfx_ctx* ctx, double* out) {
  DFX_CHECK_ARG(ctx && out, "bad argument");
  Context* c = &ctx->c;
  double h[2];
  unsigned long long lv[2];
  DFX_HIP(hipMemcpyAsync(h, &c->ds->sum_u, sizeof(h), hipMemcpyDeviceToHost, c->stream));
  DFX_HIP(hipMemcpyAsync(lv, &c->ds->live_keys, sizeof(lv), hipMemcpyDeviceToHost, c->stream));
  DFX_HIP(hipStreamSynchronize(c->stream));
  const double n = h[1] > 0 ? h[1] : 1;
  out[0] = h[0] / n;
  out[1] = (double)lv[0] / n;
  out[2] = (double)lv[1] / n;
  DFX_HIP(hipMemsetAsync(&c->ds->sum_u, 0, sizeof(h), c->stream));
  DFX_HIP(hipMemsetAsync(&c->ds->live_keys, 0, sizeof(lv), c->stream));
  if (c->loc_stream) DFX_HIP(hipStreamSynchronize(c->loc_stream));
  out[3] = 0;
  for (DevState* s : c->bds) {
    if (!s) continue;
    unsigned m = 0;
    DFX_HIP(hipMemcpy(&m, &s->lb_map_steps, sizeof(unsigned), hipMemcpyDeviceToHost));
    DFX_HIP(hipMemset(&s->lb_map_steps, 0, sizeof(unsigned)));
    out[3] += (double)m;
  }
  DFX_HIP(hipStreamSynchronize(c->stream));
  return DFX_OK;
}

extern "C" int dfx_prof_host(dfx_ctx* ctx, double* out) {
  DFX_CHECK_ARG(ctx && out, "bad argument");
  out[0] = ctx->c.host_wait_s;
  out[1] = (double)ctx->c.host_waits;
  ctx->c.host_wait_s = 0;
  ctx->c.host_waits = 0;
  return DFX_OK;
}

extern "C" int dfx_prof_lanes(dfx_ctx* ctx, double* out) {
  DFX_CHECK_ARG(ctx && out, "bad argument");
  for (int i = 0; i < 4; ++i) out[i] = ctx->c.lane_stats[i];
  return DFX_OK;
}

extern "C" int dfx_prof_read(dfx_ctx* ctx, double* ms, int* n_steps, double* mean_u) {
  DFX_CHECK_ARG(ctx && ms, "bad argument");
  Context* c = &ctx->c;
  DFX_HIP(hipStreamSynchronize(c->stream));
  for (int m = 0; m < kProfMarks - 1; ++m) ms[m] = 0;
  for (int s = 0; s < c->prof_n; ++s) {
    for (int m = 0; m < kProfMarks - 1; ++m) {
      if ((c->prof_mask >> m & 3u) != 3u) continue;
      float t = 0;
      DFX_HIP(hipEventElapsedTime(&t, c->prof_ev[(size_t)s * kProfMarks + m],
                                  c->prof_ev[(size_t)s * kProfMarks + m + 1]));
      ms[m] += t;
    }
  }
  for (double& v : c->lane_stats) v = 0;
  if (c->loc_stream) DFX_HIP(hipStreamSynchronize(c->loc_stream));
  if (c->aux_stream) DFX_HIP(hipStreamSynchronize(c->aux_stream));
  const bool lanes = (c->prof_mask >> kProfMarks & 1u) && (c->prof_mask & 1u);
  for (int s = 0; s < c->prof_n && !c->lane_ev.empty() && lanes; ++s) {
    hipEvent_t* L = &c->lane_ev[(size_t)s * 4];
    hipEvent_t* M = &c->prof_ev[(size_t)s * kProfMarks];
    float t[4] = {0, 0, 0, 0};
    DFX_HIP(hipEventElapsedTime(&t[0], L[0], L[1]));
    DFX_HIP(hipEventElapsedTime(&t[1], M[0], L[0]));
    DFX_HIP(hipEventElapsedTime(&t[2], M[0], L[1]));
    DFX_HIP(hipEventElapsedTime(&t[3], L[2], L[3]));
    for (int i = 0; i < 4; ++i) c->lane_stats[i] += t[i] / c->prof_n;
  }
  if (n_steps) *n_steps = c->prof_n;
  c->prof_n = 0;
  double h[2];
  DFX_HIP(hipMemcpyAsync(h, &c->ds->sum_u, sizeof(h), hipMemcpyDeviceToHost, c->stream));
  DFX_HIP(hipStreamSynchronize(c->stream));
  if (mean_u) *mean_u = h[1] > 0 ? h[0] / h[1] : 0;
  DFX_HIP(hipMemsetAsync(&c->ds->sum_u, 0, sizeof(h), c->stream));
  DFX_HIP(hipMemsetAsync(&c->ds->live_keys, 0, 2 * sizeof(unsigned long long), c->stream));
  DFX_HIP(hipStreamSynchronize(c->stream));
  return DFX_OK;
}
```

### difacto_amd/hotpath.py

```python
import ctypes

import numpy as np
import torch

from . import _lib
from ._lib import check

kFeaCount, kWeight, kGradient = 1, 2, 3
kTraining, kValidation, kPrediction = 3, 4, 5
MAX_INDEX = (1 << 64) - 1


def _p(t):
    return None if t is None else ctypes.c_void_p(t.data_ptr())


def _kwstr(kwargs):
    return ",".join("%s=%s" % (k, v) for k, v in kwargs.items()).encode()


class Context:

    def __init__(self, device=0, **kwargs):
        self.device = torch.device("cuda", device)
        self.kwargs = dict(kwargs)
        h = ctypes.c_void_p()
        check(_lib.lib().dfx_ctx_create(device, _kwstr(dict(kwargs, strict=1)), ctypes.byref(h)))
        self.h = h
        self.V_dim = _lib.lib().dfx_ctx_vdim(h)
        self.use_current_stream()

    def use_current_stream(self):
        s = torch.cuda.current_stream(self.device)
        check(_lib.lib().dfx_ctx_set_stream(self.h, ctypes.c_void_p(s.cuda_stream)))

    def set_input_stream(self, stream):
        check(_lib.lib().dfx_ctx_set_input_stream(
            self.h, None if stream is None else ctypes.c_void_p(stream.cuda_stream)))

    def close(self):
        if getattr(self, "h", None):
            _lib.lib().dfx_ctx_destroy(self.h)
            self.h = None

    def __del__(self):
        try:
            self.close()
        except Exception:
            pass

    def sync(self):
        check(_lib.lib().dfx_sync(self.h))

    def reserve(self, max_rows, max_nnz):
        check(_lib.lib().dfx_reserve(self.h, int(max_rows), int(max_nnz)))

    def tensor(self, a, dtype):
        if a is None:
            return None
        a = np.ascontiguousarray(a)
        if a.dtype == np.uint64:
            a = a.view(np.int64)
        elif a.dtype == np.uint32:
            a = a.view(np.int32)
        return torch.from_numpy(a.copy()).to(self.device, dtype=dtype)


class DeviceRowBlock:

    def __init__(self, ctx, blk):
        self.size = blk.size
        self.nnz = blk.nnz
        self.offs = ctx.tensor(blk.offs, torch.int64)
        self.ids = ctx.tensor(blk.ids, torch.int64)
        self.vals = ctx.tensor(blk.vals, torch.float32)
        self.labels = ctx.tensor(blk.labels, torch.float32)
        self.weights = ctx.tensor(blk.weights, torch.float32)

    def as_batch(self):
        return _lib.Batch(self.size, self.nnz, _p(self.offs), _p(self.ids), _p(self.vals),
                          _p(self.labels), _p(self.weights))


def u64(t):
    return t.cpu().numpy().view(np.uint64)


def u32(t):
    return t.cpu().numpy().view(np.uint32)


class Localizer:

    def __init__(self, ctx, max_index=MAX_INDEX):
        self.ctx = ctx
        self.max_index = max_index

    def compact(self, dblk, want_cnt=True):
        ctx = self.ctx
        nnz = dblk.nnz
        uniq = torch.empty(max(nnz, 1), dtype=torch.int64, device=ctx.device)
        cnt = torch.empty(max(nnz, 1), dtype=torch.float32, device=ctx.device) if want_cnt else None
        col = torch.empty(max(nnz, 1), dtype=torch.int32, device=ctx.device)
        n = ctypes.c_int64(0)
        check(_lib.lib().dfx_localize(ctx.h, dblk.size, nnz, _p(dblk.offs), _p(dblk.ids),
                                      ctypes.c_uint64(self.max_index), _p(uniq), _p(cnt),
                                      _p(col), ctypes.byref(n)))
        U = n.value
        return col[:nnz], uniq[:U], (cnt[:U] if want_cnt else None)


class FMLoss:

    def __init__(self, ctx, V_dim=0):
        self.ctx = ctx
        self.V_dim = int(V_dim)

    def predict(self, dblk, col, weights, w_pos, V_pos, pred, n_cols):
        check(_lib.lib().dfx_fm_predict(self.ctx.h, dblk.size, dblk.nnz, _p(dblk.offs), _p(col),
                                        _p(dblk.vals), _p(weights), _p(w_pos), _p(V_pos),
                                        int(n_cols), self.V_dim, _p(pred)))

    def calc_grad(self, dblk, col, weights, w_pos, V_pos, pred, grad, n_cols):
        check(_lib.lib().dfx_fm_calcgrad(self.ctx.h, dblk.size, dblk.nnz, _p(dblk.offs), _p(col),
                                         _p(dblk.vals), _p(dblk.labels), _p(dblk.weights),
                                         _p(weights), _p(w_pos), _p(V_pos), int(n_cols),
                                         self.V_dim, _p(pred), _p(grad)))

    def evaluate(self, label, pred):
        out = ctypes.c_double(0)
        check(_lib.lib().dfx_evaluate(self.ctx.h, pred.numel(), _p(label), _p(pred),
                                      ctypes.byref(out)))
        return out.value


def auc(ctx, label, pred):
    out = ctypes.c_double(0)
    check(_lib.lib().dfx_auc(ctx.h, pred.numel(), _p(label), _p(pred), ctypes.byref(out)))
    return out.value


def get_pos(ctx, lens):
    n = lens.numel()
    w = torch.empty(max(n, 1), dtype=torch.int32, device=ctx.device)
    v = torch.empty(max(n, 1), dtype=torch.int32, device=ctx.device)
    check(_lib.lib().dfx_get_pos(ctx.h, n, _p(lens), _p(w), _p(v)))
    return w[:n], v[:n]


class Store:

    def __init__(self, ctx):
        self.ctx = ctx

    def pull(self, keys):
        ctx = self.ctx
        n = keys.numel()
        d = ctx.V_dim
        vals = torch.empty(max(n * (1 + d), 1), dtype=torch.float32, device=ctx.device)
        lens = torch.empty(max(n, 1), dtype=torch.int32, device=ctx.device) if d > 0 else None
        nv = ctypes.c_int64(0)
        check(_lib.lib().dfx_store_pull(ctx.h, _p(keys), n, _p(vals), _p(lens), ctypes.byref(nv)))
        return vals[:nv.value], (lens[:n] if d > 0 else None)

    def push(self, keys, val_type, vals, lens=None):
        check(_lib.lib().dfx_store_push(self.ctx.h, _p(keys), keys.numel(), int(val_type),
                                        _p(vals), vals.numel(), _p(lens)))

    def save(self, path, save_aux=True):
        check(_lib.lib().dfx_store_save(self.ctx.h, str(path).encode(), int(save_aux)))

    def load(self, path):
        check(_lib.lib().dfx_store_load(self.ctx.h, str(path).encode()))

    def dump(self, path, dump_aux=False, need_reverse=False):
        check(_lib.lib().dfx_store_dump(self.ctx.h, str(path).encode(), int(dump_aux),
                                        int(need_reverse)))

    def stats(self):
        nk, nv, nw = ctypes.c_int64(0), ctypes.c_int64(0), ctypes.c_double(0)
        seed = ctypes.c_uint32(0)
        check(_lib.lib().dfx_store_stats(self.ctx.h, ctypes.byref(nk), ctypes.byref(nv),
                                         ctypes.byref(nw), ctypes.byref(seed)))
        return {"n_keys": nk.value, "n_vrows": nv.value, "new_w": nw.value, "seed": seed.value}

    def evaluate(self):
        pen, nnz = ctypes.c_double(0), ctypes.c_int64(0)
        check(_lib.lib().dfx_store_evaluate(self.ctx.h, ctypes.byref(pen), ctypes.byref(nnz)))
        return pen.value, nnz.value

    def probe_stats(self):
        m, mx, cap = ctypes.c_double(0), ctypes.c_int64(0), ctypes.c_int64(0)
        check(_lib.lib().dfx_store_probe_stats(self.ctx.h, ctypes.byref(m), ctypes.byref(mx),
                                               ctypes.byref(cap)))
        return m.value, mx.value, cap.value

    def reserve(self, n_keys, n_vrows):
        check(_lib.lib().dfx_store_reserve(self.ctx.h, int(n_keys), int(n_vrows)))

    def entry(self, key):
        d = self.ctx.V_dim
        st = (ctypes.c_float * 4)()
        V = (ctypes.c_float * max(2 * d, 1))()
        hv, found = ctypes.c_int(0), ctypes.c_int(0)
        check(_lib.lib().dfx_store_entry(self.ctx.h, ctypes.c_uint64(int(key)), st, V,
                                         ctypes.byref(hv), ctypes.byref(found)))
        if not found.value:
            return None
        return (np.array(st, np.float32),
                np.array(V, np.float32)[:2 * d].copy() if hv.value else None)


def train_step(ctx, dblk, job_type=kTraining, push_cnt=False, max_index=MAX_INDEX, pred=None):
    b = dblk.as_batch()
    check(_lib.lib().dfx_train_step(ctx.h, ctypes.byref(b), int(job_type), int(bool(push_cnt)),
                                    ctypes.c_uint64(max_index), _p(pred)))


PHASES = ("localize", "probe_pull", "feacnt", "forward", "eval_auc", "backward_update", "initv")


def prof_enable(ctx, max_steps, phases=None):
    if phases is None:
        check(_lib.lib().dfx_prof_enable(ctx.h, int(max_steps)))
        return
    mask = 0
    for p in phases:
        m = PHASES.index(p)
        mask |= 3 << m
    check(_lib.lib().dfx_prof_enable_marks(ctx.h, int(max_steps), mask))


def prof_read(ctx):
    ms = (ctypes.c_double * 7)()
    n = ctypes.c_int(0)
    mu = ctypes.c_double(0)
    check(_lib.lib().dfx_prof_read(ctx.h, ms, ctypes.byref(n), ctypes.byref(mu)))
    return dict(zip(PHASES, list(ms))), n.value, mu.value


def prof_counts(ctx):
    out = (ctypes.c_double * 4)()
    check(_lib.lib().dfx_prof_counts(ctx.h, out))
    r = dict(zip(("U", "U_V", "occ_V"), list(out)))
    r["lb_map_steps"] = int(out[3])
    return r


def prof_host(ctx):
    out = (ctypes.c_double * 2)()
    if not hasattr(_lib.lib(), "dfx_prof_host"):
        return {"wait_s": 0.0, "waits": 0}
    check(_lib.lib().dfx_prof_host(ctx.h, out))
    return {"wait_s": out[0], "waits": int(out[1])}


def prof_lanes(ctx):
    out = (ctypes.c_double * 4)()
    check(_lib.lib().dfx_prof_lanes(ctx.h, out))
    return dict(zip(("loc_ms", "loc_start_rel_ms", "loc_end_rel_ms", "auc_ms"), list(out)))


def progress(ctx, reset=True):
    p = _lib.Progress()
    check(_lib.lib().dfx_progress_read(ctx.h, ctypes.byref(p), int(reset)))
    return {"nrows": p.nrows, "loss": p.loss, "auc": p.auc, "penalty": p.penalty,
            "nnz_w": p.nnz_w}
```

### include/difacto_amd.h

```cpp
#ifndef DIFACTO_AMD_H_
#define DIFACTO_AMD_H_

#include <stddef.h>
#include <stdint.h>

#ifdef __cplusplus
extern "C" {
#endif

#define DFX_OK 0
#define DFX_ERR_ARG 1
#define DFX_ERR_HIP 2
#define DFX_ERR_CAPACITY 3
#define DFX_ERR_CHECK 4
#define DFX_ERR_IO 5

#define DFX_FEA_COUNT 1
#define DFX_WEIGHT 2
#define DFX_GRADIENT 3

#define DFX_JOB_TRAINING 3
#define DFX_JOB_VALIDATION 4
#define DFX_JOB_PREDICTION 5

typedef struct dfx_ctx dfx_ctx;

typedef struct dfx_batch {
  int64_t size;
  int64_t nnz;
  const uint64_t* offset;
  const uint64_t* index;
  const float* value;
  const float* label;
  const float* weight;
} dfx_batch;

typedef struct dfx_progress {
  double nrows;
  double loss;
  double auc;
  double penalty;
  double nnz_w;
} dfx_progress;

const char* dfx_last_error(void);
int dfx_ctx_create(int device, const char* kwargs, dfx_ctx** out);
int dfx_ctx_destroy(dfx_ctx* ctx);
int dfx_ctx_set_stream(dfx_ctx* ctx, void* hip_stream);
int dfx_ctx_use_own_stream(dfx_ctx* ctx);
int dfx_ctx_lane_stream(dfx_ctx* ctx, int which, void** out);
int dfx_ctx_set_lane_stream(dfx_ctx* ctx, int which, void* hip_stream);
int dfx_ctx_set_input_stream(dfx_ctx* ctx, void* hip_stream);
int dfx_ctx_vdim(dfx_ctx* ctx);
int dfx_sync(dfx_ctx* ctx);
int dfx_malloc(dfx_ctx* ctx, void** ptr, size_t bytes);
int dfx_free(dfx_ctx* ctx, void* ptr);
int dfx_memcpy(dfx_ctx* ctx, void* dst, const void* src, size_t bytes, int kind);
int dfx_reserve(dfx_ctx* ctx, int64_t max_rows, int64_t max_nnz);

typedef struct dfx_feeder dfx_feeder;
typedef struct dfx_host_batch {
  uint64_t* offset;
  uint64_t* index;
  float* value;
  float* label;
  float* weight;
  int64_t max_rows;
  int64_t max_nnz;
} dfx_host_batch;
int dfx_feeder_create(dfx_ctx* ctx, int64_t max_rows, int64_t max_nnz, dfx_feeder** out);
int dfx_feeder_destroy(dfx_feeder* f);
int dfx_feeder_slot(dfx_feeder* f, dfx_host_batch* hb);
int dfx_feeder_submit(dfx_feeder* f, int64_t B, int64_t nnz, int has_value, int has_weight,
                      dfx_batch* out);
int dfx_feeder_consumed(dfx_feeder* f);
int dfx_feeder_create_slots(dfx_ctx* ctx, int64_t max_rows, int64_t max_nnz, int nslots,
                            dfx_feeder** out);
int dfx_feeder_consumed_back(dfx_feeder* f, int back);

int dfx_localize(dfx_ctx* ctx, int64_t B, int64_t nnz, const uint64_t* offset,
                 const uint64_t* index, uint64_t max_index, uint64_t* uniq, float* cnt,
                 uint32_t* col, int64_t* n_uniq);

int dfx_fm_predict(dfx_ctx* ctx, int64_t B, int64_t nnz, const uint64_t* offset,
                   const uint32_t* col, const float* value, const float* weights,
                   const int32_t* w_pos, const int32_t* V_pos, int64_t n_cols, int V_dim,
                   float* pred);
int dfx_fm_calcgrad(dfx_ctx* ctx, int64_t B, int64_t nnz, const uint64_t* offset,
                    const uint32_t* col, const float* value, const float* label,
                    const float* row_weight, const float* weights, const int32_t* w_pos,
                    const int32_t* V_pos, int64_t n_cols, int V_dim, const float* pred,
                    float* grad);
int dfx_get_pos(dfx_ctx* ctx, int64_t n, const int32_t* lens, int32_t* w_pos, int32_t* V_pos);
int dfx_evaluate(dfx_ctx* ctx, int64_t B, const float* label, const float* pred, double* objv);
int dfx_auc(dfx_ctx* ctx, int64_t B, const float* label, const float* pred, double* auc_n);

int dfx_store_pull(dfx_ctx* ctx, const uint64_t* keys, int64_t n, float* vals, int32_t* lens,
                   int64_t* n_vals);
int dfx_store_push(dfx_ctx* ctx, const uint64_t* keys, int64_t n, int type, const float* vals,
                   int64_t n_vals, const int32_t* lens);
int dfx_store_save(dfx_ctx* ctx, const char* path, int save_aux);
int dfx_store_load(dfx_ctx* ctx, const char* path);
int dfx_store_load_part(dfx_ctx* ctx, const char* path, int rank, int nranks);
int dfx_store_dump(dfx_ctx* ctx, const char* path, int dump_aux, int need_reverse);
int dfx_store_stats(dfx_ctx* ctx, int64_t* n_keys, int64_t* n_vrows, double* new_w,
                    uint32_t* seed);
int dfx_store_probe_stats(dfx_ctx* ctx, double* mean_probe, int64_t* max_probe,
                          int64_t* capacity);
int dfx_store_evaluate(dfx_ctx* ctx, double* penalty, int64_t* nnz);
int dfx_store_reserve(dfx_ctx* ctx, int64_t n_keys, int64_t n_vrows);
int dfx_store_entry(dfx_ctx* ctx, uint64_t key, float* state, float* V, int* has_v,
                    int* found);

int dfx_train_step(dfx_ctx* ctx, const dfx_batch* batch, int job_type, int push_cnt,
                   uint64_t max_index, float* pred_out);
int dfx_progress_read(dfx_ctx* ctx, dfx_progress* out, int reset);

int dfx_prof_enable(dfx_ctx* ctx, int max_steps);
int dfx_prof_enable_marks(dfx_ctx* ctx, int max_steps, unsigned mask);
int dfx_prof_read(dfx_ctx* ctx, double* ms, int* n_steps, double* mean_u);
int dfx_prof_lanes(dfx_ctx* ctx, double* out);
int dfx_prof_counts(dfx_ctx* ctx, double* out);
int dfx_prof_host(dfx_ctx* ctx, double* out);

int dfx_dist_record_floats(dfx_ctx* ctx);
int dfx_dist_localize(dfx_ctx* ctx, const dfx_batch* batch, uint64_t max_index, int nranks,
                      int slot, uint64_t* keys_out, float* cnt_out);
int dfx_dist_localize_wait(dfx_ctx* ctx, int slot, int nranks, int64_t* split_counts,
                           int64_t* n_uniq);
int dfx_dist_owner_begin(dfx_ctx* ctx, int slot, const uint64_t* recv_keys,
                         const int64_t* recv_offsets, int nranks, const float* recv_cnt);
int dfx_dist_owner_pull(dfx_ctx* ctx, int slot, float* vals_out);
int dfx_dist_fwd_bwd(dfx_ctx* ctx, int slot, const dfx_batch* batch, const float* pulled,
                     int job_type, float* grads_out, float* pred_out);
int dfx_dist_owner_push(dfx_ctx* ctx, int slot, const float* recv_grads);
int dfx_dist_initv_local(dfx_ctx* ctx, int slot, int64_t* count_dev);
int dfx_dist_initv_draw(dfx_ctx* ctx, int slot, const int64_t* counts_all_dev, int rank,
                        int nranks);
int dfx_dist_push_agg_sum(dfx_ctx* ctx);
int dfx_dist_union(dfx_ctx* ctx, const uint64_t* runs, const int64_t* run_offs, int nruns,
                   int nranks, uint64_t* union_out, uint32_t* upos_out, int64_t* bounds_out,
                   int64_t* n_union);
int dfx_dist_union_rows(dfx_ctx* ctx, const uint64_t* keys, const uint32_t* upos, int64_t U,
                        const int64_t* bounds, int nranks, int64_t M, int width, int to_union,
                        const float* src, float* dst);

int dfx_split_part_floats(dfx_ctx* ctx, int nranks);
int dfx_split_pxv_floats(dfx_ctx* ctx);
int dfx_split_partition(dfx_ctx* ctx, int slot, const dfx_batch* batch, uint64_t max_index,
                        int nranks, uint64_t* keys_out, float* x_out, uint32_t* row_cnt_out);
int dfx_split_partition_wait(dfx_ctx* ctx, int slot, int nranks, int64_t* split_counts);
int dfx_split_owner_begin(dfx_ctx* ctx, int slot, const uint64_t* keys, const float* x,
                          uint32_t* row_cnt, const int64_t* rows_per_rank,
                          const int64_t* keys_per_rank, int nranks, int job_type,
                          int push_cnt, int lane);
int dfx_split_owner_forward(dfx_ctx* ctx, int slot, float* part_out);
int dfx_split_combine(dfx_ctx* ctx, int slot, const dfx_batch* batch, const float* parts,
                      int64_t part_rows, int nranks, float* pxv_out, float* pred_out);
int dfx_split_owner_backward(dfx_ctx* ctx, int slot, const float* pxv);
int dfx_split_owner_forward_rows(dfx_ctx* ctx, int slot, float* part_out, int nranks, int64_t M,
                                 int64_t lo, int64_t len);
int dfx_split_combine_rows(dfx_ctx* ctx, int slot, const dfx_batch* batch, const float* parts,
                           int64_t part_rows, int nranks, float* pxv_out, float* pred_out,
                           int64_t lo, int64_t len);
int dfx_split_owner_stats(dfx_ctx* ctx, int slot, int64_t* rows, int64_t* nnz,
                          int64_t* n_uniq);
int dfx_split_initv_local(dfx_ctx* ctx, int slot, int64_t* count_dev);
int dfx_split_initv_draw(dfx_ctx* ctx, int slot, const int64_t* counts_all_dev, int rank,
                         int nranks);

#ifdef __cplusplus
}
#endif
#endif
```

Baseline: 139.3 million train examples/sec.

## Pack localize bucket items into 32-bit words when key range fits

Adds a 32-bit item form for the bucketed localize sort: when the key range relative to each bucket's lower bound plus the row index fits in 31 bits, scatter writes uint32 items instead of uint64, and the per-bucket wave sort, head detection and unique-key output decode full keys from the bucket base. This halves scatter/sort traffic and LDS footprint and skips the high radix passes. It also removes diagnostic tiling/mid4 paths from the scatter kernel and adds a profiling counter for how often the 32-bit path runs. The choice depends on the previous step's hint, so a mismatch between steps is handled by falling back through lb_over and the global path, which adds branching complexity.

```diff
diff --git a/difacto_amd/_lib.py b/difacto_amd/_lib.py
--- a/difacto_amd/_lib.py
+++ b/difacto_amd/_lib.py
@@ -44,6 +44,7 @@
     "dfx_prof_lanes": (ctypes.c_int, [vp, f64p]),
     "dfx_prof_counts": (ctypes.c_int, [vp, f64p]),
     "dfx_prof_host": (ctypes.c_int, [vp, f64p]),
+    "dfx_prof_lb_w32": (ctypes.c_int, [vp, f64p]),
     "dfx_ctx_vdim": (ctypes.c_int, [vp]),
     "dfx_sync": (ctypes.c_int, [vp]),
     "dfx_malloc": (ctypes.c_int, [vp, ctypes.POINTER(vp), ctypes.c_size_t]),
diff --git a/difacto_amd/csrc/internal.h b/difacto_amd/csrc/internal.h
--- a/difacto_amd/csrc/internal.h
+++ b/difacto_amd/csrc/internal.h
@@ -78,6 +78,9 @@
   unsigned int lb_nhot, lb_hm_n, lb_hm_s;
   unsigned int lb_map_steps;
   unsigned long long lb_hm_base;
+  unsigned int lb_w32, lb_w32_s;
+  unsigned int lb_w32_steps;
+  unsigned long long lb_w32_base;
   alignas(128) unsigned long long bw_stripe[kBwStripes][16];
 };
 
diff --git a/difacto_amd/csrc/lb_item.h b/difacto_amd/csrc/lb_item.h
--- /dev/null
+++ b/difacto_amd/csrc/lb_item.h
@@ -0,0 +1,76 @@
+#pragma once
+#include <stdint.h>
+
+#if defined(__HIPCC__)
+#define DFX_HD __host__ __device__
+#else
+#define DFX_HD
+#endif
+
+namespace dfx {
+
+DFX_HD inline int lb_bitlen(uint64_t x) {
+  return x ? 64 - __builtin_clzll((unsigned long long)x) : 0;
+}
+
+struct LbMap {
+  uint64_t base;
+  int s;
+  uint32_t nbk;
+};
+DFX_HD inline uint32_t lb_bucket(uint64_t k, const LbMap& m) {
+  if (k <= m.base) return 0u;
+  const uint64_t x = (k - m.base) >> m.s;
+  return x < m.nbk ? (uint32_t)x : m.nbk - 1u;
+}
+
+struct LbItem {
+  uint64_t kmin, kmax;
+  int lo, rb;
+};
+
+DFX_HD inline uint64_t lb_f(const LbItem& p, uint64_t k) { return (k - p.kmin) >> p.lo; }
+
+DFX_HD inline uint64_t lb_least(const LbItem& p, const LbMap& m, uint32_t b) {
+  if (b == 0) return p.kmin;
+  const uint64_t off = (uint64_t)b << m.s;
+  uint64_t L = m.base + off;
+  if ((off >> m.s) != (uint64_t)b || L < m.base) L = ~0ull;
+  return L > p.kmin ? L : p.kmin;
+}
+
+DFX_HD inline uint64_t lb_maxrel(const LbItem& p, const LbMap& m) {
+  const uint64_t span = (1ull << m.s) - 1;
+  uint64_t top0 = p.kmax;
+  if (m.nbk > 1) {
+    uint64_t t = m.base + span;
+    if (t < m.base) t = ~0ull;
+    top0 = t < top0 ? t : top0;
+  }
+  uint64_t r = top0 >= p.kmin ? lb_f(p, top0) : 0;
+  if (m.nbk > 2) {
+    const uint64_t in = (span >> p.lo) + 1;
+    r = in > r ? in : r;
+  }
+  if (m.nbk > 1) {
+    const uint64_t L = lb_least(p, m, m.nbk - 1);
+    if (p.kmax >= L) {
+      const uint64_t x = lb_f(p, p.kmax) - lb_f(p, L);
+      r = x > r ? x : r;
+    }
+  }
+  return r;
+}
+
+DFX_HD inline bool lb_fits32(const LbItem& p, const LbMap& m) {
+  return p.kmin <= p.kmax && p.rb + lb_bitlen(lb_maxrel(p, m)) <= 31;
+}
+
+DFX_HD inline uint32_t lb_item32(const LbItem& p, uint64_t k, uint64_t q, uint64_t fb) {
+  return ((uint32_t)(lb_f(p, k) - fb) << p.rb) | (uint32_t)q;
+}
+DFX_HD inline uint64_t lb_fullkey(const LbItem& p, uint32_t item, uint64_t fb) {
+  return (((uint64_t)(item >> p.rb) + fb) << p.lo) + p.kmin;
+}
+
+}
diff --git a/difacto_amd/csrc/locbucket.hip b/difacto_amd/csrc/locbucket.hip
--- a/difacto_amd/csrc/locbucket.hip
+++ b/difacto_amd/csrc/locbucket.hip
@@ -1,7 +1,9 @@
 #include <algorithm>
 #include <mutex>
 #include <set>
-
+#include <type_traits>
+
+#include "lb_item.h"
 #include "lookback.h"
 
 namespace dfx {
@@ -65,13 +67,6 @@
   return reverse_bytes(m);
 }
 
-__device__ inline int lb_bitlen(uint64_t x) { return x ? 64 - __clzll((long long)x) : 0; }
-
-struct LbMap {
-  uint64_t base;
-  int s;
-  uint32_t nbk;
-};
 __device__ inline LbMap lb_map(const DevState* ds, int wbits) {
   LbMap m;
   m.nbk = 1u << wbits;
@@ -85,12 +80,6 @@
   }
   return m;
 }
-__device__ inline uint32_t lb_bucket(uint64_t k, const LbMap& m) {
-  if (k <= m.base) return 0u;
-  const uint64_t x = (k - m.base) >> m.s;
-  return x < m.nbk ? (uint32_t)x : m.nbk - 1u;
-}
-
 constexpr int kLbHotMax = 1024;
 struct LbHot {
   const uint64_t* hk;
@@ -150,14 +139,13 @@
   return c + h.hp[i];
 }
 
-struct LbPack {
-  uint64_t kmin;
-  int lo, rb;
+struct LbPack : LbItem {
   bool packed;
 };
 __device__ inline LbPack lb_pack(const DevState* ds, uint64_t qmax) {
   LbPack p;
   p.kmin = ds->kmin;
+  p.kmax = ds->kmax;
   const uint64_t diff = ds->or_mask ^ ds->and_mask;
   p.lo = diff ? __ffsll((long long)diff) - 1 : 0;
   p.rb = lb_bitlen(qmax);
@@ -166,6 +154,15 @@
 }
 __device__ inline uint64_t lb_keybits(const LbPack& p, uint64_t it) {
   return p.packed ? it >> p.rb : it;
+}
+
+constexpr int kLbLdsPacked = 0, kLbLdsQ = 1, kLbLds32 = 2;
+__device__ inline LbMap lb_map32(const DevState* ds, int wbits) {
+  LbMap m;
+  m.nbk = 1u << wbits;
+  m.base = ds->lb_w32_base;
+  m.s = (int)ds->lb_w32_s;
+  return m;
 }
 
 __global__ void k_lb_init(DevState* ds) {
@@ -186,6 +183,14 @@
   return v;
 }
 __device__ inline unsigned long long lb_wave_and(unsigned long long v) {
+  for (int off = 32; off > 0; off >>= 1) v &= __shfl_xor(v, off, kWave);
+  return v;
+}
+__device__ inline unsigned int lb_wave_or(unsigned int v) {
+  for (int off = 32; off > 0; off >>= 1) v |= __shfl_xor(v, off, kWave);
+  return v;
+}
+__device__ inline unsigned int lb_wave_and(unsigned int v) {
   for (int off = 32; off > 0; off >>= 1) v &= __shfl_xor(v, off, kWave);
   return v;
 }
@@ -312,8 +317,9 @@
   }
 }
 
-template <bool S, int HNT, bool HOT>
+template <bool S, int HNT, bool HOT, bool W32>
 __global__ __launch_bounds__(HNT) void k_lb_scatter(LbArgs a) {
+  static_assert(!(HOT && W32), "the hot-key map's buckets are no key ranges");
   constexpr int kLbHNT = HNT, kLbHWaves = HNT / kWave;
   extern __shared__ uint64_t lb_dyn64[];
   __shared__ uint32_t lds[kLbHWaves + 1];
@@ -325,9 +331,7 @@
   const bool qs = HOT && lb_hot_on(a);
   LbHot hm{};
   if (qs) hm = lb_stage_hot(a, offs + a.rt + 1, t, kLbHNT);
-  const int64_t tile = ((a.diag & 512) && a.ntiles % 8 == 0)
-                           ? (int64_t)(blockIdx.x % 8) * (a.ntiles / 8) + blockIdx.x / 8
-                           : (int64_t)blockIdx.x;
+  const int64_t tile = blockIdx.x;
   const int64_t r0 = tile * a.rt;
   const int nr = (int)(a.B - r0 < a.rt ? a.B - r0 : a.rt);
   const uint32_t per = (m.nbk + kLbHNT - 1) / kLbHNT;
@@ -343,50 +347,31 @@
   uint32_t total;
   uint32_t ex = block_excl_scan<kLbHNT>(mine, lds, &total);
   const uint32_t* pre = a.tilecnt + (size_t)tile * m.nbk;
-  const bool mid4 = (a.diag & 512) && per == 4;
-  uint32_t msum = 0;
-  const uint32_t mex = ex;
   for (uint32_t i = 0; i < per; ++i) {
     const uint32_t d = t * per + i;
     if (d < m.nbk) {
-      if (!mid4) cur[d] = ex + pre[d];
-      msum += pre[d];
+      cur[d] = ex + pre[d];
       if (blockIdx.x == 0) a.bstart[d] = ex;
       ex += a.totals[d];
     }
   }
-  if (mid4) {
-    __syncthreads();
-    cur[t] = mex + msum;
-  }
-  if (a.diag & 256) {
-    auto tcnt = [&](uint32_t d) {
-      const uint32_t nx = tile + 1 < a.ntiles ? a.tilecnt[(size_t)(tile + 1) * m.nbk + d]
-                                              : a.totals[d];
-      return nx - pre[d];
-    };
-    uint32_t lm = 0;
-    for (uint32_t i = 0; i < per; ++i)
-      if (t * per + i < m.nbk) lm += tcnt(t * per + i);
-    uint32_t lex = block_excl_scan<kLbHNT>(lm, lds, nullptr);
-    for (uint32_t i = 0; i < per; ++i) {
-      const uint32_t d = t * per + i;
-      if (d < m.nbk) {
-        const uint32_t cd = tcnt(d);
-        cur[d] = lex;
-        lex += cd;
-      }
-    }
-  }
   const uint64_t qmax = (S || a.rowof) ? (uint64_t)(a.nnz - 1) : (uint64_t)(a.B - 1);
   const LbPack p = lb_pack(a.ds, qmax);
+  const bool fit = p.packed && lb_fits32(p, m);
+  const bool w32 =
+      W32 && fit && !qs &&
+      __hip_atomic_load(&a.ds->lb_over, __ATOMIC_RELAXED, __HIP_MEMORY_SCOPE_AGENT) == 0u;
   if (blockIdx.x == 0) {
     uint32_t nover;
     (void)block_excl_scan<kLbHNT>(over, lds, &nover);
     if (t == 0) {
       a.bstart[m.nbk] = total;
       a.hint[0] = nover;
-      a.hint[2] = p.packed ? 1u : 2u;
+      a.hint[2] = !p.packed ? 2u : (fit && nover == 0u) ? 3u : 1u;
+      a.ds->lb_w32 = w32 ? 1u : 0u;
+      a.ds->lb_w32_base = m.base;
+      a.ds->lb_w32_s = (unsigned)m.s;
+      if (w32) a.ds->lb_w32_steps += 1u;
     }
   }
   for (int i = t; i <= nr; i += kLbHNT) offs[i] = a.offset[r0 + i];
@@ -437,10 +422,15 @@
       const uint32_t row = (uint32_t)(r0 + lo);
       const uint64_t q = S ? j : (uint64_t)row;
       const uint32_t bk = qs ? lb_hot_bucket(k, j, hm) : lb_bucket(k, m);
-      const uint32_t pos = atomicAdd(&cur[mid4 ? bk >> 2 : bk], 1u);
-      stnt((a.diag & 128) ? a.sscr + j : (a.diag & (256 | 512)) ? a.sscr + (a.diag & 256 ? j0 : 0) + pos : a.kbuf + pos,
-           p.packed ? ((((k - p.kmin) >> p.lo) << p.rb) | (q & qmask)) : k, a.nt != 0);
-      if (!p.packed) a.qbuf[pos] = (uint32_t)q;
+      const uint32_t pos = atomicAdd(&cur[bk], 1u);
+      if (W32 && w32) {
+        stnt(reinterpret_cast<uint32_t*>(a.kbuf) + pos,
+             lb_item32(p, k, q & qmask, lb_f(p, lb_least(p, m, bk))), a.nt != 0);
+      } else {
+        stnt(a.kbuf + pos, p.packed ? ((((k - p.kmin) >> p.lo) << p.rb) | (q & qmask)) : k,
+             a.nt != 0);
+        if (!p.packed) a.qbuf[pos] = (uint32_t)q;
+      }
       if (S && a.rowof) a.rowof[j] = make_uint2(row, __float_as_uint(x[u]));
       else if (S) a.sbuf[pos] = (uint64_t)__float_as_uint(x[u]) | ((uint64_t)row << 32);
     }
@@ -646,12 +636,12 @@
   }
 }
 
-__device__ inline bool lb_needs_global(int64_t n, bool packed, int q_lds) {
-  return n > kLbCap || (!packed && !q_lds);
+__device__ inline bool lb_needs_global(int64_t n, bool packed, int form, bool w32) {
+  return n > kLbCap || (form == kLbLds32 ? !w32 : (!packed && form == kLbLdsPacked));
 }
 
 template <bool S>
-__global__ __launch_bounds__(kLbNT) void k_lb_big(LbArgs a, int q_lds) {
+__global__ __launch_bounds__(kLbNT) void k_lb_big(LbArgs a, int form) {
   __shared__ uint32_t wcnt[kLbWaves][256];
   __shared__ uint32_t base[256];
   __shared__ uint32_t lds[kLbWaves + 1];
@@ -661,8 +651,9 @@
   const uint64_t qmax = (S || a.rowof) ? (uint64_t)(a.nnz - 1) : (uint64_t)(a.B - 1);
   const LbPack p = lb_pack(a.ds, qmax);
   const bool hasq = !p.packed;
+  const bool w32 = a.ds->lb_w32 != 0u;
   if (__hip_atomic_load(&a.ds->lb_over, __ATOMIC_RELAXED, __HIP_MEMORY_SCOPE_AGENT) == 0u &&
-      (p.packed || q_lds))
+      !lb_needs_global(0, p.packed, form, w32))
     return;
   __shared__ uint32_t s_list[kLbNT];
   __shared__ uint32_t s_nlist;
@@ -670,7 +661,7 @@
   for (uint32_t b0 = 0; b0 < nbk; b0 += kLbNT) {
     const uint32_t bb = b0 + t;
     const int64_t nb = bb < nbk ? (int64_t)a.bstart[bb + 1] - (int64_t)a.bstart[bb] : 0;
-    const uint32_t need = (bb < nbk && nb > 1 && lb_needs_global(nb, p.packed, q_lds)) ? 1u : 0u;
+    const uint32_t need = (bb < nbk && nb > 1 && lb_needs_global(nb, p.packed, form, w32)) ? 1u : 0u;
     uint32_t cnt;
     const uint32_t ex = block_excl_scan<kLbNT>(need, lds, &cnt);
     if (t == 0) s_nlist = 0;
@@ -745,27 +736,33 @@
 constexpr int kLbWIT = kLbCap / kWave;
 
 
-template <bool Q, bool S>
+template <bool Q, bool S, typename T>
 __device__ __attribute__((always_inline)) inline void lb_wave_sort(
-    const uint64_t* gk, const uint32_t* gq, const uint64_t* gs, int n, bool hasq, int ntp,
-    int diag, uint64_t* sk, uint32_t* sq, uint64_t* ss, uint32_t* cnt) {
+    const T* gk, const uint32_t* gq, const uint64_t* gs, int n, bool hasq, int ntp,
+    int diag, T* sk, uint32_t* sq, uint64_t* ss, uint32_t* cnt) {
+  static_assert(!Q || sizeof(T) == 8, "a 32-bit item carries its q");
+  using W = typename std::conditional<sizeof(T) == 8, unsigned long long, unsigned int>::type;
+  constexpr T kPad = ~(T)0;
+  constexpr int kPasses = 4 + (int)sizeof(T);
   const int l = threadIdx.x;
   const int nc = (n + kWave - 1) / kWave;
-  uint64_t k[kLbWIT], sv[kLbWIT];
+  T k[kLbWIT];
+  uint64_t sv[kLbWIT];
   uint32_t q[kLbWIT];
 #pragma unroll
   for (int c = 0; c < kLbWIT; ++c) {
     const int i = c * kWave + l;
     const bool v = c < nc && i < n;
-    k[c] = v ? ldnt(gk + i, ntp != 0) : ~0ull;
+    k[c] = v ? ldnt(gk + i, ntp != 0) : kPad;
     q[c] = (Q && hasq) ? (v ? gq[i] : ~0u) : 0u;
     sv[c] = (S && v) ? gs[i] : 0ull;
   }
-  unsigned long long kor = 0, kand = ~0ull, qor = 0, qand = ~0ull;
+  W kor = 0, kand = ~(W)0;
+  unsigned long long qor = 0, qand = ~0ull;
 #pragma unroll
   for (int c = 0; c < kLbWIT; ++c) {
     if (c < nc) {
-      kor |= k[c] == ~0ull ? 0ull : k[c];
+      kor |= k[c] == kPad ? (T)0 : k[c];
       kand &= k[c];
       if (Q && hasq) {
         qor |= q[c] == ~0u ? 0u : q[c];
@@ -788,7 +785,7 @@
     };
     int last = -1;
     if (!(diag & 1))
-      for (int pass = 0; pass < 12; ++pass) {
+      for (int pass = Q ? 0 : 4; pass < kPasses; ++pass) {
         bool on_q;
         int shift;
         if (!pass_at(pass, &on_q, &shift)) break;
@@ -805,7 +802,7 @@
         }
       }
     }
-    for (int pass = 0; pass <= last; ++pass) {
+    for (int pass = Q ? 0 : 4; pass <= last; ++pass) {
       bool on_q;
       int shift;
       (void)pass_at(pass, &on_q, &shift);
@@ -881,9 +878,11 @@
   passes();
 }
 
-template <bool Q, bool S>
+template <bool Q, bool S, bool W32>
 __global__ __launch_bounds__(kWave) void k_lb_wbucket(LbArgs a) {
-  __shared__ uint64_t sk[kLbCap];
+  static_assert(!(Q && W32), "a 32-bit item carries its q");
+  using T = typename std::conditional<W32, uint32_t, uint64_t>::type;
+  __shared__ T sk[kLbCap];
   __shared__ uint32_t sq[Q ? kLbCap : 1];
   __shared__ uint64_t ss[S ? kLbCap : 1];
   __shared__ uint32_t cnt[256];
@@ -895,37 +894,46 @@
   const uint64_t qmax = (S || a.rowof) ? (uint64_t)(a.nnz - 1) : (uint64_t)(a.B - 1);
   const LbPack p = lb_pack(ds, qmax);
   const bool hasq = !p.packed;
-  const bool fast = !lb_needs_global(n, p.packed, Q ? 1 : 0);
+  const bool w32 = W32 && ds->lb_w32 != 0u;
+  const bool fast =
+      !lb_needs_global(n, p.packed, W32 ? kLbLds32 : Q ? kLbLdsQ : kLbLdsPacked, w32);
   const uint64_t* gk = a.kbuf + start;
   const uint32_t* gq = a.qbuf + start;
   const uint64_t* gs = a.sbuf + start;
   const int nc = (n + kWave - 1) / kWave;
   if (fast)
-    lb_wave_sort<Q, S>(gk, gq, gs, n, hasq, a.nt, a.diag, sk, sq, ss, cnt);
+    lb_wave_sort<Q, S, T>(reinterpret_cast<const T*>(a.kbuf) + start, gq, gs, n, hasq, a.nt,
+                          a.diag, sk, sq, ss, cnt);
+  const uint64_t fb = w32 ? lb_f(p, lb_least(p, lb_map32(ds, a.wbits), b)) : 0ull;
   const uint64_t qmask = p.rb ? (~0ull >> (64 - p.rb)) : 0ull;
   uint32_t* tseg = a.qscr + start;
   uint64_t* tkey = a.kscr + start;
+  uint32_t* tkey32 = reinterpret_cast<uint32_t*>(a.kscr) + start;
   uint32_t run = 0;
   bool longseg = false, hot = false;
   const int th = (int)a.hot_th;
   auto fullkey = [&](uint64_t it) { return p.packed ? (((it >> p.rb) << p.lo) + p.kmin) : it; };
-  auto heads = [&](const uint64_t* K, const uint32_t* Qs, const uint64_t* Ss) {
-    uint64_t prev = 0;
+  auto heads = [&](auto K, const uint32_t* Qs, const uint64_t* Ss) {
+    using I = typename std::remove_cv<typename std::remove_pointer<decltype(K)>::type>::type;
+    constexpr bool k32 = sizeof(I) == 4;
+    auto keybits = [&](I x) { return k32 ? (I)(x >> p.rb) : (I)lb_keybits(p, x); };
+    I prev = 0;
     for (int c = 0; c < nc; ++c) {
       const int i = c * kWave + l;
       const bool valid = i < n;
-      const uint64_t it = valid ? K[i] : 0ull;
-      const uint64_t kb = lb_keybits(p, it);
-      const uint64_t up = __shfl_up(kb, 1, kWave);
+      const I it = valid ? K[i] : (I)0;
+      const I kb = keybits(it);
+      const I up = __shfl_up(kb, 1, kWave);
       const bool h = valid && (i == 0 || kb != (l == 0 ? prev : up));
-      if (valid && i >= kChunkOcc && kb == lb_keybits(p, K[i - kChunkOcc])) longseg = true;
-      if (longseg && valid && i >= th && kb == lb_keybits(p, K[i - th])) hot = true;
+      if (valid && i >= kChunkOcc && kb == keybits(K[i - kChunkOcc])) longseg = true;
+      if (longseg && valid && i >= th && kb == keybits(K[i - th])) hot = true;
       prev = __shfl(kb, kWave - 1, kWave);
       const uint64_t hb = __ballot(h);
       if (!(a.diag & 4) && valid) {
         if (h) {
           const uint32_t r = run + (uint32_t)__popcll(hb & lanemask_lt());
-          tkey[r] = fullkey(it);
+          if (k32) tkey32[r] = (uint32_t)it;
+          else tkey[r] = fullkey(it);
           tseg[r] = (uint32_t)(start + i);
         }
         uint32_t row;
@@ -933,21 +941,24 @@
           const uint64_t sw = Ss[i];
           row = (uint32_t)(sw >> 32);
           if (a.occ_x) a.occ_x[start + i] = __uint_as_float((uint32_t)sw);
-        } else if (a.rowof) {
-          row = p.packed ? (uint32_t)(it & qmask) : Qs[i];
         } else {
-          row = p.packed ? (uint32_t)(it & qmask) : Qs[i];
+          row = (k32 || p.packed) ? (uint32_t)(it & (I)qmask) : Qs[i];
         }
         a.occ_row[start + i] = row;
       }
       run += (uint32_t)__popcll(hb);
     }
   };
-  if (fast) heads(sk, sq, ss);
+  if (fast) heads((const T*)sk, sq, ss);
   else heads(gk, gq, gs);
   if (n > 0 && l == 0) {
-    a.bfk[b] = fullkey(fast ? sk[0] : gk[0]);
-    a.blk[b] = fullkey(fast ? sk[n - 1] : gk[n - 1]);
+    if (W32 && fast) {
+      a.bfk[b] = lb_fullkey(p, (uint32_t)sk[0], fb);
+      a.blk[b] = lb_fullkey(p, (uint32_t)sk[n - 1], fb);
+    } else {
+      a.bfk[b] = fullkey(fast ? (uint64_t)sk[0] : gk[0]);
+      a.blk[b] = fullkey(fast ? (uint64_t)sk[n - 1] : gk[n - 1]);
+    }
   }
   if (__ballot(hot) && l == 0 &&
       __hip_atomic_load(&ds->lb_hot, __ATOMIC_RELAXED, __HIP_MEMORY_SCOPE_AGENT) == 0u)
@@ -1019,6 +1030,17 @@
   const uint32_t b = blockIdx.x;
   const int64_t start = a.bstart[b];
   const uint32_t h = a.bheads[b], r0 = a.brank[b], c = a.bcont[b];
+  if (a.ds->lb_w32) {
+    const uint64_t qmax = (a.value || a.rowof) ? (uint64_t)(a.nnz - 1) : (uint64_t)(a.B - 1);
+    const LbPack p = lb_pack(a.ds, qmax);
+    const uint64_t fb = lb_f(p, lb_least(p, lb_map32(a.ds, a.wbits), b));
+    const uint32_t* it = reinterpret_cast<const uint32_t*>(a.kscr) + start;
+    for (uint32_t j = threadIdx.x + c; j < h; j += kLbNT) {
+      if (a.uniq) a.uniq[r0 + j - c] = lb_fullkey(p, it[j], fb);
+      if (a.segstart) a.segstart[r0 + j - c] = a.qscr[start + j];
+    }
+    return;
+  }
   for (uint32_t j = threadIdx.x + c; j < h; j += kLbNT) {
     if (a.uniq) a.uniq[r0 + j - c] = a.kscr[start + j];
     if (a.segstart) a.segstart[r0 + j - c] = a.qscr[start + j];
@@ -1215,7 +1237,7 @@
   a.uniq = o.uniq; a.segstart = o.segstart; a.occ_row = o.occ_row;
   a.occ_x = valued ? o.occ_x : nullptr;
   a.hint = ws.lb_hint;
-  a.diag = (c->lb_diag & ~(16 | 32 | 64 | 128 | 256 | 512)) | c->lb_skip;
+  a.diag = (c->lb_diag & ~(16 | 32 | 64 | 128 | 256 | 512)) | (c->lb_skip & (16 | 32 | 64));
   {
     constexpr size_t kNb = (size_t)1 << kLbMaxBits;
     char* q = ws.lbsplit.as<char>();
@@ -1253,39 +1275,44 @@
                      L.stream, a);
   const size_t scatter_lds =
       ((nbk + 1) & ~1u) * sizeof(uint32_t) + (rt + 1) * sizeof(uint64_t) + sp_bytes;
+  const unsigned form_hint = hint[2];
+  const bool q_lds = form_hint == 2u;
+  const bool w32 = form_hint == 3u && !hm_lds;
+#define DFX_LB_SCAT1(S, NT, HOT, W)                                                        \
+  {                                                                                        \
+    lb_lds_attr((const void*)k_lb_scatter<S, NT, HOT, W>);                                 \
+    hipLaunchKernelGGL((k_lb_scatter<S, NT, HOT, W>), dim3((unsigned)ntiles), dim3(NT),     \
+                       scatter_lds, L.stream, a);                                          \
+  }
 #define DFX_LB_SCAT(NT)                                                                    \
-  lb_lds_attr((const void*)k_lb_scatter<true, NT, false>);                                 \
-  lb_lds_attr((const void*)k_lb_scatter<false, NT, false>);                                \
-  lb_lds_attr((const void*)k_lb_scatter<false, NT, true>);                                 \
-  if (valued)                                                                              \
-    hipLaunchKernelGGL((k_lb_scatter<true, NT, false>), dim3((unsigned)ntiles), dim3(NT),   \
-                       scatter_lds, L.stream, a);                                          \
-  else if (a.hm_lds)                                                                       \
-    hipLaunchKernelGGL((k_lb_scatter<false, NT, true>), dim3((unsigned)ntiles), dim3(NT),   \
-                       scatter_lds, L.stream, a);                                          \
-  else                                                                                     \
-    hipLaunchKernelGGL((k_lb_scatter<false, NT, false>), dim3((unsigned)ntiles), dim3(NT),  \
-                       scatter_lds, L.stream, a);
+  if (valued && w32) DFX_LB_SCAT1(true, NT, false, true)                                   \
+  else if (valued) DFX_LB_SCAT1(true, NT, false, false)                                    \
+  else if (a.hm_lds) DFX_LB_SCAT1(false, NT, true, false)                                  \
+  else if (w32) DFX_LB_SCAT1(false, NT, false, true)                                       \
+  else DFX_LB_SCAT1(false, NT, false, false)
   if (c->lb_skip & 16) {}
   else if (hnt == 256) { DFX_LB_SCAT(256) }
   else if (hnt == 512) { DFX_LB_SCAT(512) }
   else { DFX_LB_SCAT(1024) }
 #undef DFX_LB_SCAT
-  const bool q_lds = hint[2] == 2u;
+#undef DFX_LB_SCAT1
+  const int form = w32 ? kLbLds32 : q_lds ? kLbLdsQ : kLbLdsPacked;
   const dim3 bg(nbk), bb(kLbNT);
   const bool carry = valued && !gather;
   if (carry)
-    hipLaunchKernelGGL(k_lb_big<true>, dim3(kLbBigBlocks), bb, 0, L.stream, a, q_lds ? 1 : 0);
+    hipLaunchKernelGGL(k_lb_big<true>, dim3(kLbBigBlocks), bb, 0, L.stream, a, form);
   else
-    hipLaunchKernelGGL(k_lb_big<false>, dim3(kLbBigBlocks), bb, 0, L.stream, a, q_lds ? 1 : 0);
+    hipLaunchKernelGGL(k_lb_big<false>, dim3(kLbBigBlocks), bb, 0, L.stream, a, form);
   const dim3 wb(kWave);
   if (c->lb_skip & 32) {}
   else if (carry) {
-    if (q_lds) hipLaunchKernelGGL((k_lb_wbucket<true, true>), bg, wb, 0, L.stream, a);
-    else hipLaunchKernelGGL((k_lb_wbucket<false, true>), bg, wb, 0, L.stream, a);
+    if (w32) hipLaunchKernelGGL((k_lb_wbucket<false, true, true>), bg, wb, 0, L.stream, a);
+    else if (q_lds) hipLaunchKernelGGL((k_lb_wbucket<true, true, false>), bg, wb, 0, L.stream, a);
+    else hipLaunchKernelGGL((k_lb_wbucket<false, true, false>), bg, wb, 0, L.stream, a);
   } else {
-    if (q_lds) hipLaunchKernelGGL((k_lb_wbucket<true, false>), bg, wb, 0, L.stream, a);
-    else hipLaunchKernelGGL((k_lb_wbucket<false, false>), bg, wb, 0, L.stream, a);
+    if (w32) hipLaunchKernelGGL((k_lb_wbucket<false, false, true>), bg, wb, 0, L.stream, a);
+    else if (q_lds) hipLaunchKernelGGL((k_lb_wbucket<true, false, false>), bg, wb, 0, L.stream, a);
+    else hipLaunchKernelGGL((k_lb_wbucket<false, false, false>), bg, wb, 0, L.stream, a);
   }
   const bool defer = gather && c->lb_gather == 2 && o.rowof_out != nullptr;
   if (o.rowof_out) *o.rowof_out = defer ? a.rowof : nullptr;
diff --git a/difacto_amd/csrc/step.hip b/difacto_amd/csrc/step.hip
--- a/difacto_amd/csrc/step.hip
+++ b/difacto_amd/csrc/step.hip
@@ -389,6 +389,22 @@
   return DFX_OK;
 }
 
+extern "C" int dfx_prof_lb_w32(dfx_ctx* ctx, double* out) {
+  DFX_CHECK_ARG(ctx && out, "bad argument");
+  Context* c = &ctx->c;
+  DFX_HIP(hipStreamSynchronize(c->stream));
+  if (c->loc_stream) DFX_HIP(hipStreamSynchronize(c->loc_stream));
+  out[0] = 0;
+  for (DevState* s : c->bds) {
+    if (!s) continue;
+    unsigned m = 0;
+    DFX_HIP(hipMemcpy(&m, &s->lb_w32_steps, sizeof(unsigned), hipMemcpyDeviceToHost));
+    DFX_HIP(hipMemset(&s->lb_w32_steps, 0, sizeof(unsigned)));
+    out[0] += (double)m;
+  }
+  return DFX_OK;
+}
+
 extern "C" int dfx_prof_host(dfx_ctx* ctx, double* out) {
   DFX_CHECK_ARG(ctx && out, "bad argument");
   out[0] = ctx->c.host_wait_s;
diff --git a/difacto_amd/hotpath.py b/difacto_amd/hotpath.py
--- a/difacto_amd/hotpath.py
+++ b/difacto_amd/hotpath.py
@@ -244,6 +244,11 @@
     check(_lib.lib().dfx_prof_counts(ctx.h, out))
     r = dict(zip(("U", "U_V", "occ_V"), list(out)))
     r["lb_map_steps"] = int(out[3])
+    r["lb_w32_steps"] = 0
+    if hasattr(_lib.lib(), "dfx_prof_lb_w32"):
+        w = (ctypes.c_double * 1)()
+        check(_lib.lib().dfx_prof_lb_w32(ctx.h, w))
+        r["lb_w32_steps"] = int(w[0])
     return r
 
 
diff --git a/include/difacto_amd.h b/include/difacto_amd.h
--- a/include/difacto_amd.h
+++ b/include/difacto_amd.h
@@ -122,6 +122,7 @@
 int dfx_prof_lanes(dfx_ctx* ctx, double* out);
 int dfx_prof_counts(dfx_ctx* ctx, double* out);
 int dfx_prof_host(dfx_ctx* ctx, double* out);
+int dfx_prof_lb_w32(dfx_ctx* ctx, double* out);
 
 int dfx_dist_record_floats(dfx_ctx* ctx);
 int dfx_dist_localize(dfx_ctx* ctx, const dfx_batch* batch, uint64_t max_index, int nranks,
```

Measured after the change: 142.6 million train examples/sec (median of 6 runs). +2.4%, better.
